# jean-pierreBoth/gsearch

Measured on AMD Instinct MI355X. Metric: query genomes/sec, higher is better.
Workload: dtype f32

## Files before the change

### gsearch_amd/csrc/gs_index.hip

```cpp
#include <algorithm>
#include <functional>
#include <chrono>
#include <math.h>
#include <memory>
#include <stdlib.h>
#include <string.h>
#include <vector>
#include <sys/stat.h>
#include "gs_internal.hpp"
#include "gs_spec.hpp"
#include "gs_insert_rows.hpp"
#include "gs_hnswio_parse.hpp"

namespace gs {

constexpr int ST = 1024;
constexpr int SMAXI = 16;
constexpr int RIF = 8;
#define KEY(c, id) (((uint64_t)(c) << 32) | (uint64_t)(id))
#define KCNT(k) ((uint32_t)((k) >> 32))
#define KID(k) ((uint32_t)(k))
#define INF_CNT 0xFFFFFFFFu

struct IndexDev {
// ... 1877 lines not shown
        list_ptrs(g, list, nbr, cnt, deg, cap);
        const uint32_t d = *deg, ni = inbox_cnt[list], n = d + ni;
        __syncthreads();
        for (uint32_t t = threadIdx.x; t < n; t += LM_T)
            keys[t] = t < d ? KEY(cnt[t], nbr[t]) : inbox[(uint64_t)list * inbox_cap + (t - d)];
        bool unsorted = false;
        for (uint32_t t = threadIdx.x + 1; t < d; t += LM_T) unsorted |= !(keys[t - 1] < keys[t]);
        const bool general = __syncthreads_or(unsorted) != 0;
        uint32_t rk[LM_MAX / LM_T]; uint64_t kv[LM_MAX / LM_T];
        uint32_t ndup = 0;
        if (general) {
            for (uint32_t t = threadIdx.x; t < n; t += LM_T) {
                const uint64_t k = keys[t]; uint32_t dup = 0;
                for (uint32_t j = 0; j < t; j++) dup |= (keys[j] == k);
                flag[t] = dup;
            }
            __syncthreads();
#pragma unroll
            for (int it = 0; it < LM_MAX / LM_T; it++) {
                const uint32_t t = threadIdx.x + it * LM_T;
                rk[it] = 0xFFFFFFFFu; kv[it] = 0;
                if (t < n && !flag[t]) {
                    const uint64_t k = keys[t]; uint32_t r = 0;
                    for (uint32_t j = 0; j < n; j++) r += (!flag[j] && keys[j] < k);
                    rk[it] = r; kv[it] = k;
                }
            }
            for (uint32_t j = 0; j < n; j++) ndup += flag[j];
        } else {
            for (uint32_t u = threadIdx.x; u < ni; u += LM_T) {
                const uint64_t k = keys[d + u];
                uint32_t lo = 0, hi = d;
                while (lo < hi) { const uint32_t mid = (lo + hi) >> 1; if (keys[mid] < k) lo = mid + 1; else hi = mid; }
                uint32_t dup = lo < d && keys[lo] == k;
                for (uint32_t v = 0; v < u; v++) dup |= (keys[d + v] == k);
                flag[d + u] = dup | (lo << 1);
            }
            __syncthreads();
#pragma unroll
            for (int it = 0; it < LM_MAX / LM_T; it++) {
                const uint32_t t = threadIdx.x + it * LM_T;
                rk[it] = 0xFFFFFFFFu; kv[it] = 0;
                if (t < d) {
                    const uint64_t k = keys[t]; uint32_t r = t;
                    for (uint32_t v = 0; v < ni; v++) r += (!(flag[d + v] & 1u) && keys[d + v] < k);
                    rk[it] = r; kv[it] = k;
                } else if (t < n && !(flag[t] & 1u)) {
                    const uint64_t k = keys[t]; uint32_t r = flag[t] >> 1;
                    for (uint32_t v = 0; v < ni; v++) r += (!(flag[d + v] & 1u) && keys[d + v] < k);
                    rk[it] = r; kv[it] = k;
                }
            }
            for (uint32_t v = 0; v < ni; v++) ndup += flag[d + v] & 1u;
        }
        __syncthreads();
#pragma unroll
        for (int it = 0; it < LM_MAX / LM_T; it++) if (rk[it] < cap) { nbr[rk[it]] = KID(kv[it]); cnt[rk[it]] = KCNT(kv[it]); }
        if (threadIdx.x == 0) { const uint32_t tot = n - ndup; *deg = tot < cap ? tot : cap; inbox_cnt[list] = 0; }
    }
}

}

struct gs_index {
    gs_ctx *ctx = nullptr;
    gs_index_params prm{};
    size_t esz = 4, rowbytes = 0; uint64_t stride = 0; uint32_t nchunks = 0;
    int ikind = GS_KIND_F32; size_t user_rowbytes = 0;
    uint64_t n = 0, cap = 0; int64_t entry = -1; int top = -1;
    uint64_t n_upper = 0, cap_upper = 0;
    gs::DevBuf data;
    gs::DevBuf levels;
    gs::DevBuf deg0;
    gs::DevBuf nbr0;
    gs::DevBuf cnt0;
    gs::DevBuf upidx;
    gs::DevBuf degU;
    gs::DevBuf nbrU;
    gs::DevBuf cntU;
    gs::DevBuf visited;
    gs::DevBuf counter;
    gs::DevBuf cbuf;
    gs::DevBuf blevels;
    gs::DevBuf cntmat;
    gs::DevBuf plan_keys;
    gs::DevBuf plan_n;
    gs::DevBuf inbox;
    gs::DevBuf inbox_cnt;
    gs::DevBuf touched;
    gs::DevBuf ntouched;
    gs::DevBuf evals_dev;
    gs::DevBuf wlog;
    gs::DevBuf w0_keys;
    gs::DevBuf w0_n;
    gs::DevBuf w0_evals;
    gs::DevBuf ep0;
    gs::DevBuf ext_keys;
    uint64_t inbox_lists = 0;
    uint64_t insert_evals = 0;
    gs::DevBuf mat;
    double search_frac = -1.0, insert_frac = -1.0;
    gs::DevBuf cols; uint64_t cols_cap = 0, cols_n = 0;
    gs::DevBuf join_scratch[gs::JOIN_SCRATCH];
    gs::DevBuf stats;
    uint64_t stat_wg_in_flight = 0, stat_adj_row_bytes = 0;
    gs::DevBuf rowptr;
    gs::DevBuf sp_off, sp_meta, sp_bm, sp_arena; uint32_t sp_L = 0; bool sp_tried = false;
    gs::VmArena sp_vm;
    bool sp_exhausted = false;
    uint64_t sp_reserved = 0;
    std::vector<std::unique_ptr<gs::DevBuf>> slabs;
    gs::DevBuf *call_slab = nullptr;
    gs::DevBuf *early_rows = nullptr;
    uint64_t pair_cache_bytes = 0, pair_cache_budget = 0;
    std::vector<uint64_t> origin;
    std::vector<int32_t> pid_rank;
    uint64_t level_count[17] = {0};
    gs::DevBuf origin_d, pid_rank_d; uint64_t origin_d_n = 0, pid_rank_d_n = 0;
    std::function<int(uint64_t, uint64_t)> *feed = nullptr; const uint8_t *feed_base = nullptr;
};

namespace gs {

static std::vector<DevBuf *> index_scratch(gs_index *ix)
{
    std::vector<DevBuf *> v = {&ix->visited, &ix->counter, &ix->cbuf, &ix->blevels, &ix->cntmat, &ix->plan_keys, &ix->plan_n, &ix->inbox, &ix->touched, &ix->ntouched,
                               &ix->wlog, &ix->w0_keys, &ix->w0_n, &ix->w0_evals, &ix->ep0, &ix->ext_keys, &ix->mat};
    for (DevBuf &b : ix->join_scratch) v.push_back(&b);
    return v;
}

static void ids_append(gs_index *ix, const uint64_t *ids, const uint8_t *lv, uint64_t n);

static void drop_pair_cache(gs_index *ix)
{
    (void)hipGetLastError();
    if (!ix->slabs.empty()) {
        (void)hipStreamSynchronize(ix->ctx->stream);
        if (ix->rowptr.p) (void)hipMemsetAsync(ix->rowptr.p, 0, ix->rowptr.bytes, ix->ctx->stream);
        (void)hipStreamSynchronize(ix->ctx->stream);
        ix->slabs.clear();
    }
    ix->call_slab = ix->early_rows = nullptr;
    ix->pair_cache_bytes = 0; ix->pair_cache_budget = 1;
}
static int alloc_or_evict(gs_index *ix, DevBuf &b, size_t bytes)
{
    int rc = b.alloc(bytes);
    if (rc == GS_OK || (ix->slabs.empty() && ix->pair_cache_budget == 1)) return rc;
    drop_pair_cache(ix);
    return b.alloc(bytes);
}

static int index_reserve(gs_index *ix, uint64_t need, uint64_t need_upper)
{
    gs_ctx *c = ix->ctx;
    const uint32_t M = ix->prm.max_nb_conn, ML = ix->prm.max_layer;
    if (need > ix->cap) {
        uint64_t ncap = std::max<uint64_t>(need, std::max<uint64_t>(ix->cap + ix->cap / 2, 1024));
        if (ix->prm.capacity >= need && ncap > ix->prm.capacity) ncap = ix->prm.capacity;
        if (ix->cols.p && (uint64_t)ix->stride * ncap > ((uint64_t)8 << 30)) { ix->cols.release(); ix->cols_cap = 0; ix->cols_n = 0; }
        struct Arr { DevBuf *b; size_t per; };
        std::vector<Arr> arr = {
            {&ix->data, (size_t)ix->stride}, {&ix->levels, 1}, {&ix->deg0, 4}, {&ix->nbr0, (size_t)8 * M}, {&ix->cnt0, (size_t)8 * M}, {&ix->upidx, 4}, {&ix->rowptr, 8}};
        if (ix->sp_L && ix->sp_meta.p) { arr.push_back({&ix->sp_off, 4}); arr.push_back({&ix->sp_meta, 8}); arr.push_back({&ix->sp_bm, 8}); }
        for (auto &a : arr) {
            DevBuf nb;
            int rc = alloc_or_evict(ix, nb, a.per * ncap); if (rc) return rc;
            GS_HIP_CHECK(hipMemsetAsync(nb.p, 0, a.per * ncap, c->stream));
            if (ix->n) GS_HIP_CHECK(hipMemcpyAsync(nb.p, a.b->p, a.per * ix->n, hipMemcpyDeviceToDevice, c->stream));
            GS_HIP_CHECK(hipStreamSynchronize(c->stream));
            std::swap(a.b->p, nb.p); std::swap(a.b->bytes, nb.bytes);
        }
        ix->cap = ncap;
    }
    if (need_upper > ix->cap_upper) {
        uint64_t ncap = std::max<uint64_t>(need_upper, std::max<uint64_t>(ix->cap_upper * 2, 64));
        struct { DevBuf *b; size_t per; } arr[] = {{&ix->degU, (size_t)4 * ML}, {&ix->nbrU, (size_t)4 * ML * M}, {&ix->cntU, (size_t)4 * ML * M}};
        for (auto &a : arr) {
            DevBuf nb;
            int rc = nb.alloc(a.per * ncap); if (rc) return rc;
            GS_HIP_CHECK(hipMemsetAsync(nb.p, 0, a.per * ncap, c->stream));
            if (ix->n_upper) GS_HIP_CHECK(hipMemcpyAsync(nb.p, a.b->p, a.per * ix->n_upper, hipMemcpyDeviceToDevice, c->stream));
            GS_HIP_CHECK(hipStreamSynchronize(c->stream));
            std::swap(a.b->p, nb.p); std::swap(a.b->bytes, nb.bytes);
        }
        ix->cap_upper = ncap;
    }
    return GS_OK;
}

static IndexDev index_dev(const gs_index *ix)
{
    IndexDev d;
    d.data = ix->data.as<uint8_t>(); d.stride = ix->stride; d.nchunks = ix->nchunks; d.m = ix->prm.m;
    d.M = ix->prm.max_nb_conn; d.max_layer = ix->prm.max_layer;
    d.levels = ix->levels.as<uint8_t>(); d.deg0 = ix->deg0.as<uint32_t>(); d.nbr0 = ix->nbr0.as<uint32_t>();
    d.upidx = ix->upidx.as<int32_t>(); d.degU = ix->degU.as<uint32_t>(); d.nbrU = ix->nbrU.as<uint32_t>();
    d.rowptr = ix->rowptr.as<uint64_t>();
    const bool sp = ix->sp_L && ix->sp_meta.p;
    d.sp_base = sp ? (const uint8_t *)ix->sp_vm.va : nullptr; d.sp_off = sp ? ix->sp_off.as<uint32_t>() : nullptr; d.sp_meta = sp ? ix->sp_meta.as<uint64_t>() : nullptr; d.sp_L = sp ? ix->sp_L : 0;
    d.sp_bm = sp ? ix->sp_bm.as<uint64_t>() : nullptr;
    d.n = ix->n; d.entry = ix->entry; d.top = ix->top;
    return d;
}

static int upload_rows(gs_ctx *c, void *dst, uint64_t stride, const void *src, size_t rowbytes, uint64_t nrows, hipMemcpyKind kind)
{
    if (nrows == 0) return GS_OK;
    GS_HIP_CHECK(hipMemsetAsync(dst, 0, stride * nrows, c->stream));
    GS_HIP_CHECK(hipMemcpy2DAsync(dst, stride, src, rowbytes, rowbytes, nrows, kind, c->stream));
    return GS_OK;
}

static int upload_user_rows(gs_index *ix, void *dst, const void *src, uint64_t nrows, hipMemcpyKind kind)
{
    gs_ctx *c = ix->ctx;
    if (ix->prm.kind != GS_KIND_U16) return upload_rows(c, dst, ix->stride, src, ix->rowbytes, nrows, kind);
    if (nrows == 0) return GS_OK;
    GS_HIP_CHECK(hipMemsetAsync(dst, 0, ix->stride * nrows, c->stream));
    const void *dev = src;
    PoolBuf stage(c, SL_IX_ROW_STAGE);
    if (kind == hipMemcpyHostToDevice) {
        int rc = stage.alloc(ix->user_rowbytes * nrows); if (rc) return rc;
        GS_HIP_CHECK(hipMemcpyAsync(stage.p, src, ix->user_rowbytes * nrows, hipMemcpyHostToDevice, c->stream));
        dev = stage.p;
    }
    return widen_u16_rows(c, dev, nrows, ix->prm.m, dst, ix->stride);
}
static int download_user_rows(gs_index *ix, uint64_t first, uint64_t n, void *out_host)
{
    gs_ctx *c = ix->ctx;
    if (n == 0) return GS_OK;
    if (ix->prm.kind != GS_KIND_U16) {
        GS_HIP_CHECK(hipMemcpy2DAsync(out_host, ix->rowbytes, ix->data.as<uint8_t>() + first * ix->stride, ix->stride, ix->rowbytes, n, hipMemcpyDeviceToHost, c->stream));
    } else {
        PoolBuf stage(c, SL_IX_ROW_STAGE);
        int rc = stage.alloc(ix->user_rowbytes * n); if (rc) return rc;
        if ((rc = narrow_u16_rows(c, ix->data.as<uint8_t>() + first * ix->stride, ix->stride, n, ix->prm.m, stage.p))) return rc;
        GS_HIP_CHECK(hipMemcpyAsync(out_host, stage.p, ix->user_rowbytes * n, hipMemcpyDeviceToHost, c->stream));
    }
    GS_HIP_CHECK(hipStreamSynchronize(c->stream));
    return GS_OK;
}

enum DistMode { MODE_AUTO = 0, MODE_GATHER = 1, MODE_DENSE = 2 };
static DistMode env_mode()
{
    const char *e = getenv("GS_DIST_MODE");
    if (!e) return MODE_AUTO;
    if (!strcmp(e, "gather")) return MODE_GATHER;
    if (!strcmp(e, "dense")) return MODE_DENSE;
    return MODE_AUTO;
}
static bool use_join(const gs_index *ix);
static bool dense_pays(const gs_index *ix, double frac, uint64_t nq)
{
    const double rc = ix->ctx->rel_compute, rh = ix->ctx->rel_hbm;
    const double n = (double)ix->n, q = (double)std::max<uint64_t>(nq, 1), evals = frac * n;
    const double gather = evals * (double)ix->rowbytes * std::max(q / (5.5e12 * rh), 1.0 / (8.0e10 * rh));
    double dense;
    if (use_join(ix)) dense = n * (double)ix->rowbytes / ((nq <= 512 ? 3.5e12 : 1.0e12) * rc) * std::ceil(q / (double)match_join_max_queries()) + 3e-3;
    else dense = std::ceil(q / 128.0) * 128.0 * n * (double)ix->prm.m / ((ix->ikind == GS_KIND_U64 ? 1.4e13 : 1.6e13) * rc);
    dense += evals * 75e-9 / rc * std::max(1.0, q / 768.0);
    return dense < gather;
}
static bool use_join(const gs_index *ix)
{
    const char *e = getenv("GS_DENSE_IMPL");
    if (e && !strcmp(e, "tile")) return false;
    return ix->prm.m <= 65535;
}
static int ensure_cols(gs_index *ix, uint64_t upto)
{
    gs_ctx *c = ix->ctx;
    int rc;
    if (ix->cols_cap != ix->cap || !ix->cols.p) {
        if ((rc = alloc_or_evict(ix, ix->cols, (size_t)ix->prm.m * ix->cap * ix->esz))) return rc;
        ix->cols_cap = ix->cap; ix->cols_n = 0;
    }
    if (ix->cols_n < upto) {
        if ((rc = rows_to_cols(c, ix->ikind, ix->prm.m, ix->data.as<uint8_t>() + ix->cols_n * ix->stride, ix->stride, upto - ix->cols_n, ix->cols.p, ix->cols_cap, ix->cols_n))) return rc;
        ix->cols_n = upto;
    }
    return GS_OK;
}
static int ensure_stats(gs_index *ix)
{
    if (ix->stats.p) return GS_OK;
    int rc = ix->stats.alloc(128);
    if (rc) return rc;
    GS_HIP_CHECK(hipMemsetAsync(ix->stats.p, 0, 128, ix->ctx->stream));
    return GS_OK;
}
static int dense_counts(gs_index *ix, const uint8_t *qrows, uint64_t nq, uint64_t n, uint16_t *out16, uint64_t ld)
{
    gs_ctx *c = ix->ctx;
    int rc;
    if (!use_join(ix))
        return hamming_qxc_strided(c, ix->ikind, ix->prm.m, qrows, nq, ix->stride, ix->data.p, n, ix->stride, nullptr, nullptr, out16, ld);
    if ((rc = ensure_cols(ix, n))) return rc;
    if ((rc = ensure_stats(ix))) return rc;
    const uint64_t parts = (nq + match_join_max_queries() - 1) / match_join_max_queries(), jq = (nq + parts - 1) / parts;
    for (uint64_t q0 = 0; q0 < nq; q0 += jq) {
        const uint64_t nb = std::min<uint64_t>(jq, nq - q0);
        int declined = 0;
        if (ix->feed && (rc = (*ix->feed)((uint64_t)(qrows - ix->feed_base) / ix->stride + q0, nb))) return rc;
        if ((rc = match_join_counts(c, ix->ikind, ix->prm.m, qrows + q0 * ix->stride, ix->stride, nb, ix->cols.p, ix->cols_cap, n, out16 + q0 * ld, ld, ix->join_scratch,
                                    &declined, ix->stats.as<unsigned long long>(), true, 0, ix->data.p, ix->stride))) return rc;
        if (declined &&
            (rc = hamming_qxc_strided(c, ix->ikind, ix->prm.m, qrows + q0 * ix->stride, nb, ix->stride, ix->data.p, n, ix->stride, nullptr, nullptr, out16 + q0 * ld, ld))) return rc;
    }
    return GS_OK;
}

static int dense_counts_range(gs_index *ix, const uint8_t *qrows, uint64_t nq, uint64_t node0, uint64_t nn, uint16_t *out16, uint64_t ld)
{
    gs_ctx *c = ix->ctx;
    int rc;
    if ((rc = ensure_cols(ix, node0 + nn))) return rc;
    if ((rc = ensure_stats(ix))) return rc;
    GS_REQUIRE(nq <= match_join_max_queries(), GS_ERR_INVALID, "dense_counts_range: too many rows");
    return match_join_counts(c, ix->ikind, ix->prm.m, qrows, ix->stride, nq, (const uint8_t *)ix->cols.p + node0 * ix->esz, ix->cols_cap, nn, out16, ld, ix->join_scratch,
                             nullptr, ix->stats.as<unsigned long long>(), false, node0);
}

static bool dense_vis_in_lds(const gs_index *ix, uint32_t knbn, uint32_t maxdeg)
{
    const size_t cap = 160 * 1024 - 1024;
    const size_t l = dense_lds_bytes(ix->prm.m, knbn, maxdeg, ix->n, true, maxdeg > (uint32_t)DT / 2 ? 512u : (uint32_t)DCN);
    const char *e = getenv("GS_DENSE_VIS");
    if (e && !strcmp(e, "global")) return false;
    if (e && !strcmp(e, "lds")) return l <= cap;
    return l <= cap;
}
static uint32_t dense_split_w(const gs_index *ix, uint32_t knbn, uint32_t maxdeg, uint32_t dcn, size_t min_bytes = 0, bool many_queries = false)
{
    const char *e = getenv("GS_DENSE_VIS");
    const bool forced = e && !strcmp(e, "split");
    if (e && !forced) { if (!strcmp(e, "global") || !strcmp(e, "lds")) return 0; }
    const bool one_per_cu = many_queries && round_up(dense_lds_bytes(ix->prm.m, knbn, maxdeg, ix->n, true, dcn), 1280) > (size_t)(160 * 1024 / 2);
    if (!forced && !one_per_cu && dense_vis_in_lds(ix, knbn, maxdeg)) return 0;
    const size_t base = std::max(dense_lds_bytes(ix->prm.m, knbn, maxdeg, 0, true, dcn), min_bytes);
    int per = getenv("GS_SPLIT_PER_CU") ? std::max(1, std::min(3, atoi(getenv("GS_SPLIT_PER_CU")))) : 2;
    uint64_t w = 0;
    for (; per >= 1 && w < 1024; per--) {
        const size_t budget = (size_t)(160 * 1024 / per) / 1280 * 1280 - 64;
        w = budget > base ? ((uint64_t)(budget - base) * 8) & ~(uint64_t)1023 : 0;
    }
    if (getenv("GS_SPLIT_W")) w = std::min<uint64_t>(w, (uint64_t)std::max(1024, atoi(getenv("GS_SPLIT_W"))) & ~(uint64_t)1023);
    if (w < 1024) return 0;
    return (uint32_t)std::min<uint64_t>(w, round_up(ix->n, 1024));
}
struct DenseGeom {
    bool ok;
    bool oneg, split, vlds;
    uint32_t dcn, vis_w;
    size_t lds;
    uint32_t per_cu, scratch_words, capC, grid;
    uint32_t p2_off;
};
static DenseGeom dense_geom(const gs_index *ix, uint64_t nq, uint32_t knbn, uint32_t ef, size_t min_lds_bytes, bool many_queries, bool with_log)
{
    const gs_ctx *c = ix->ctx;
    const size_t cap = 160 * 1024 - 1024;
    const uint32_t efs = std::max(ef, knbn), maxdeg = 2 * ix->prm.max_nb_conn;
    DenseGeom g{};
    g.oneg = maxdeg > (uint32_t)DT / 2;
    g.dcn = g.oneg ? 512u : (uint32_t)DCN;
    g.vis_w = dense_split_w(ix, knbn, maxdeg, g.dcn, min_lds_bytes, many_queries);
    g.split = g.vis_w != 0;
    const bool whole = dense_vis_in_lds(ix, knbn, maxdeg);
    g.vlds = with_log || g.split || whole;
    g.lds = std::max(dense_lds_bytes(ix->prm.m, knbn, maxdeg, g.split ? (uint64_t)g.vis_w : ix->n, g.vlds, g.dcn), min_lds_bytes);
    if (with_log && g.oneg) g.ok = false;
    else if (g.split) g.ok = true;
    else if (whole) g.ok = g.lds <= cap;
    else g.ok = !with_log && g.lds <= cap;
    const size_t granted = round_up(g.lds, 1280);
    g.per_cu = (uint32_t)std::max<size_t>(1, std::min<size_t>(3, (160 * 1024) / granted));
    if (g.oneg) g.per_cu = std::min<uint32_t>(g.per_cu, 2);
    if (!with_log && getenv("GS_DENSE_PER_CU")) g.per_cu = std::max(1, std::min((int)g.per_cu, atoi(getenv("GS_DENSE_PER_CU"))));
    g.scratch_words = (g.vlds ? dense_nblocks(ix->prm.m) * (HB / 2) : (uint32_t)((ix->n + 31) / 32)) + (g.split && ix->n > g.vis_w ? (uint32_t)((ix->n - g.vis_w + 31) / 32) : 0u);
    g.capC = 2 * efs + 2 * g.dcn + maxdeg + 64;
    g.grid = (uint32_t)std::min<uint64_t>(nq, (uint64_t)c->n_cu * g.per_cu);
    g.p2_off = (getenv("GS_DENSE_PHASE2") && !atoi(getenv("GS_DENSE_PHASE2"))) ? 1u : 0u;
    return g;
}
static int search_launch_dense(gs_index *ix, uint64_t nq, uint32_t knbn, uint32_t ef, const uint16_t *mat, uint64_t mat_ld, uint64_t *ids, float *dist,
                               uint32_t *count, uint64_t *evals)
{
    gs_ctx *c = ix->ctx;
    const DenseGeom g = dense_geom(ix, nq, knbn, ef, 0, nq >= (uint64_t)2 * c->n_cu, false);
    int rc;
    if ((rc = ensure_stats(ix))) return rc;
    ix->stat_wg_in_flight = g.grid; ix->stat_adj_row_bytes = (uint64_t)8 * ix->prm.max_nb_conn + 4;
    if ((rc = ix->visited.ensure((size_t)4 * g.scratch_words * c->n_cu * 3))) return rc;
    if ((rc = ix->cbuf.ensure((size_t)16 * g.capC * c->n_cu * 3))) return rc;
    GS_HIP_CHECK(hipMemsetAsync(ix->counter.p, 0, 8, c->stream));
    IndexDev d = index_dev(ix);
    unsigned long long *prof = nullptr;
    DevBuf profbuf;
    if (getenv("GS_TRAV_PROFILE")) { if ((rc = profbuf.alloc(128))) return rc; GS_HIP_CHECK(hipMemsetAsync(profbuf.p, 0, 128, c->stream)); prof = profbuf.as<unsigned long long>(); }
    {
    ProfScope ps(c, FAM_SEARCH);
#define GS_LAUNCH_DSEARCH(V, P, O, G) GS_LAUNCH_DSEARCH_S(V, P, O, G, false)
#define GS_LAUNCH_DSEARCH_S(V, P, O, G, SP)                                                                                  \
    do {                                                                                                                  \
        auto kern = k_hnsw_search_dense<V, P, O, G, false, SP>;                                                            \
        GS_HIP_CHECK(hipFuncSetAttribute((const void *)kern, hipFuncAttributeMaxDynamicSharedMemorySize, (int)g.lds));    \
        hipLaunchKernelGGL(kern, dim3(g.grid), dim3(DT), g.lds, c->stream, d, nq, knbn, ef, mat, mat_ld, ix->visited.as<uint32_t>(), g.scratch_words, \
                           ix->cbuf.as<uint64_t>(), g.capC, ix->counter.as<unsigned long long>(), ids, dist, count, evals, prof, ix->stats.as<unsigned long long>(),  \
                           (uint64_t *)nullptr, g.p2_off, 0u, (uint64_t *)nullptr, (uint32_t *)nullptr, (const uint32_t *)nullptr, g.vis_w);  \
    } while (0)
    if (g.split) { if (g.oneg) GS_LAUNCH_DSEARCH_S(true, false, 4, true, true); else GS_LAUNCH_DSEARCH_S(true, false, 4, false, true); }
    else if (g.oneg) { if (g.vlds) GS_LAUNCH_DSEARCH(true, false, 4, true); else GS_LAUNCH_DSEARCH(false, false, 4, true); }
    else if (prof) { if (g.vlds) GS_LAUNCH_DSEARCH(true, true, 4, false); else GS_LAUNCH_DSEARCH(false, true, 4, false); }
    else if (g.per_cu >= 3) { if (g.vlds) GS_LAUNCH_DSEARCH(true, false, 6, false); else GS_LAUNCH_DSEARCH(false, false, 6, false); }
    else { if (g.vlds) GS_LAUNCH_DSEARCH(true, false, 4, false); else GS_LAUNCH_DSEARCH(false, false, 4, false); }
#undef GS_LAUNCH_DSEARCH
#undef GS_LAUNCH_DSEARCH_S
    }
    GS_HIP_CHECK(hipGetLastError());
    if (prof) {
        unsigned long long h[16];
        GS_HIP_CHECK(hipMemcpyAsync(h, prof, 128, hipMemcpyDeviceToHost, c->stream));
        GS_HIP_CHECK(hipStreamSynchronize(c->stream));
        fprintf(stderr, "[GS_TRAV_PROFILE] workgroup 0: pops %llu merges %llu | cycles/pop: loads+atomics issue->ballot %.0f, sync1 %.0f, compaction+sync2 %.0f, accept rule+count %.0f | merge cycles/merge %.0f\n",
                h[5], h[6], (double)h[0] / h[5], (double)h[1] / h[5], (double)h[2] / h[5], (double)h[3] / h[5], h[6] ? (double)h[4] / h[6] : 0.0);
        if (h[6]) fprintf(stderr, "[GS_TRAV_PROFILE] of %llu accepting pops: %llu merged into T, %llu folded N into G\n", h[6], h[13], h[14]);
        if (h[6]) fprintf(stderr, "[GS_TRAV_PROFILE] per accepting pop: compaction+sort %.0f, prefetch+trim %.0f, T %.0f, fold+N merge %.0f cycles; accepted keys %.2f\n",
                          (double)h[8] / h[6], (double)h[9] / h[6], (double)h[10] / h[6], (double)h[11] / h[6], (double)h[12] / h[6]);
    }
    return GS_OK;
}

static bool dense_traversal_fits(const gs_index *ix, uint32_t knbn, uint32_t efs)
{
    const uint32_t maxdeg = 2 * ix->prm.max_nb_conn;
    return maxdeg <= (uint32_t)DT && efs <= 65535u && knbn <= (uint32_t)(TMAXI * DT) && ix->prm.m <= 65535u &&
           dense_lds_bytes(ix->prm.m, knbn, maxdeg, ix->n, false, maxdeg > (uint32_t)DT / 2 ? 512u : (uint32_t)DCN) <= 160 * 1024 - 1024 && !getenv("GS_DENSE_LEGACY");
}
static int search_launch(gs_index *ix, const uint8_t *q_padded_dev, uint64_t nq, uint32_t knbn, uint32_t ef, const uint16_t *mat, uint64_t mat_ld,
                         uint64_t *ids, float *dist, uint32_t *count, uint64_t *evals)
{
    gs_ctx *c = ix->ctx;
    const uint32_t efs = std::max(ef, knbn);
    const uint32_t maxdeg = 2 * ix->prm.max_nb_conn;
    if (mat && dense_traversal_fits(ix, knbn, efs)) return search_launch_dense(ix, nq, knbn, ef, mat, mat_ld, ids, dist, count, evals);
    const size_t lds = search_lds_bytes(efs, maxdeg);
    const uint32_t vis_words = (uint32_t)((ix->n + 31) / 32);
    uint32_t grid = (uint32_t)std::min<uint64_t>(nq, (uint64_t)c->n_cu);
    GS_HIP_CHECK(hipMemsetAsync(ix->counter.p, 0, 8, c->stream));
    IndexDev d = index_dev(ix);
    ProfScope ps(c, FAM_SEARCH);
#define GS_LAUNCH_SEARCH(K)                                                                                               \
    do {                                                                                                                  \
        auto kern = k_hnsw_search<K>;                                                                                     \
        GS_HIP_CHECK(hipFuncSetAttribute((const void *)kern, hipFuncAttributeMaxDynamicSharedMemorySize, (int)lds));      \
        hipLaunchKernelGGL(kern, dim3(grid), dim3(ST), lds, c->stream, d, q_padded_dev, nq, knbn, ef, mat, mat_ld,       \
                           ix->visited.as<uint32_t>(), vis_words, ix->counter.as<unsigned long long>(), ids, dist, count, evals); \
    } while (0)
    if (ix->ikind == GS_KIND_F32) GS_LAUNCH_SEARCH(GS_KIND_F32);
    else if (ix->ikind == GS_KIND_U32) GS_LAUNCH_SEARCH(GS_KIND_U32);
    else GS_LAUNCH_SEARCH(GS_KIND_U64);
#undef GS_LAUNCH_SEARCH
    GS_HIP_CHECK(hipGetLastError());
    return GS_OK;
}

static bool search_goes_dense(const gs_index *ix, uint64_t nq, uint32_t knbn, uint32_t ef)
{
    const uint32_t efs = std::max(ef, knbn);
    const DistMode mode = env_mode();
    if (ix->prm.m > 65535) return false;
    if (mode == MODE_DENSE) return true;
    const bool eligible = mode == MODE_AUTO && ix->n >= 4096;
    return eligible && dense_pays(ix, (double)std::min<uint64_t>(ix->n, efs) / (double)ix->n, nq);
}
static int search_dev(gs_index *ix, const void *q_padded_dev, uint64_t nq, uint32_t knbn, uint32_t ef, uint64_t *ids, float *dist,
                      uint32_t *count, uint64_t *evals)
{
    gs_ctx *c = ix->ctx;
    const uint32_t efs = std::max(ef, knbn);
    const uint32_t maxdeg = 2 * ix->prm.max_nb_conn;
    const size_t lds = search_lds_bytes(efs, maxdeg);
    GS_REQUIRE(maxdeg <= ST, GS_ERR_UNSUPPORTED, "max_nb_conn too large");
    const DistMode mode = env_mode();
    const bool fits_sorted = lds <= 160 * 1024 - 64 && 2 * (size_t)efs + maxdeg + 64 <= (size_t)SMAXI * ST;
    const bool dense_able = mode != MODE_GATHER && dense_traversal_fits(ix, knbn, efs);
    GS_REQUIRE(fits_sorted || dense_able, GS_ERR_UNSUPPORTED, "ef=%u needs %zu bytes of LDS in the sorted-array traversal (max ~%u with M=%u) and this index / mode does not admit the dense one (m <= 65535, ef <= 65535, GS_DIST_MODE != gather)",
               efs, lds, (unsigned)((160 * 1024 - 64 - 32 * maxdeg - 1024) / 24), ix->prm.max_nb_conn);
    const bool force_dense = !fits_sorted;
    const uint32_t vis_words = (uint32_t)((ix->n + 31) / 32);
    int rc;
    if ((rc = ix->visited.ensure((size_t)4 * vis_words * c->n_cu))) return rc;
    if ((rc = ix->counter.ensure(64))) return rc;
    const uint8_t *q = (const uint8_t *)q_padded_dev;
    uint64_t done = 0;
    DevBuf tmp_evals;
    const bool eligible = mode == MODE_AUTO && ix->prm.m <= 65535 && ix->n >= 4096;
    const bool lb_dense = eligible && dense_pays(ix, (double)std::min<uint64_t>(ix->n, efs) / (double)ix->n, nq);
    if (eligible && !lb_dense && ix->search_frac < 0 && nq >= 256 && !force_dense) {
        const uint64_t np = 128;
        uint64_t *ev = evals;
        if (!ev) { if ((rc = tmp_evals.alloc(8 * np))) return rc; ev = tmp_evals.as<uint64_t>(); }
        if ((rc = search_launch(ix, q, np, knbn, ef, nullptr, 0, ids, dist, count, ev))) return rc;
        std::vector<uint64_t> h(np);
        GS_HIP_CHECK(hipMemcpyAsync(h.data(), ev, 8 * np, hipMemcpyDeviceToHost, c->stream));
        GS_HIP_CHECK(hipStreamSynchronize(c->stream));
        double sum = 0; for (uint64_t v : h) sum += (double)v;
        ix->search_frac = sum / (double)np / (double)ix->n;
        done = np;
    }
    const uint64_t rest = nq - done;
    const double frac_known = ix->search_frac >= 0 ? ix->search_frac : ix->insert_frac;
    bool dense = ix->prm.m <= 65535 && (mode == MODE_DENSE || force_dense || lb_dense || (eligible && frac_known >= 0 && rest >= 1 && dense_pays(ix, frac_known, rest)));
    if (!dense) {
        if (rest) {
            uint64_t *ev = evals ? evals + done : nullptr;
            if (!ev && eligible && ix->search_frac < 0) { if ((rc = tmp_evals.alloc(8 * rest))) return rc; ev = tmp_evals.as<uint64_t>(); }
            if ((rc = search_launch(ix, q + done * ix->stride, rest, knbn, ef, nullptr, 0, ids + done * knbn, dist + done * knbn, count ? count + done : nullptr, ev))) return rc;
            if (eligible && ix->search_frac < 0 && ev) {
                const uint64_t ns = std::min<uint64_t>(rest, 128);
                std::vector<uint64_t> h(ns);
                GS_HIP_CHECK(hipMemcpyAsync(h.data(), ev, 8 * ns, hipMemcpyDeviceToHost, c->stream));
                GS_HIP_CHECK(hipStreamSynchronize(c->stream));
                double sum = 0; for (uint64_t v : h) sum += (double)v;
                ix->search_frac = sum / (double)ns / (double)ix->n;
            }
        }
        return GS_OK;
    }
    const uint64_t ld = round_up(ix->n, 8);
    const bool join = use_join(ix);
    uint64_t budget = (uint64_t)4 << 30;
    {
        size_t fr = 0, tot = 0;
        if (hipMemGetInfo(&fr, &tot) == hipSuccess) budget = std::max<uint64_t>(budget, std::min<uint64_t>((uint64_t)32 << 30, (uint64_t)(0.7 * (double)((uint64_t)fr + ix->mat.bytes))));
    }
    uint64_t QB = budget / (2 * ld);
    QB = std::max<uint64_t>(128, QB / 128 * 128);
    if (getenv("GS_SEARCH_QB")) QB = std::min<uint64_t>(QB, (uint64_t)std::max(1, atoi(getenv("GS_SEARCH_QB"))));
    QB = std::min<uint64_t>(QB, rest);
    const bool sv = getenv("GS_SEARCH_VERBOSE") != nullptr;
    const auto sv_t0 = std::chrono::steady_clock::now();
    if (sv) { size_t fr = 0, tot = 0; (void)hipMemGetInfo(&fr, &tot); fprintf(stderr, "[GS_SEARCH] nq %llu n %llu: QB %llu, count matrix %.2f GB wanted, %.2f GB held, device free %.2f GB\n", (unsigned long long)nq, (unsigned long long)ix->n, (unsigned long long)QB, 2.0 * QB * ld / 1e9, ix->mat.bytes / 1e9, fr / 1e9); }
    if (ix->mat.bytes < (size_t)2 * QB * ld && (rc = alloc_or_evict(ix, ix->mat, (size_t)2 * QB * ld))) return rc;
    if (sv) fprintf(stderr, "[GS_SEARCH] count matrix ready after %.1f ms\n", std::chrono::duration<double, std::milli>(std::chrono::steady_clock::now() - sv_t0).count());
    if (join && (rc = ensure_cols(ix, ix->n))) return rc;
    for (uint64_t q0 = done; q0 < nq; q0 += QB) {
        const uint64_t nb = std::min(QB, nq - q0);
        if ((rc = dense_counts(ix, q + q0 * ix->stride, nb, ix->n, ix->mat.as<uint16_t>(), ld))) return rc;
        if (sv) { (void)hipStreamSynchronize(c->stream); fprintf(stderr, "[GS_SEARCH] count matrix of %llu queries done at %.1f ms\n", (unsigned long long)nb, std::chrono::duration<double, std::milli>(std::chrono::steady_clock::now() - sv_t0).count()); }
        if ((rc = search_launch(ix, q + q0 * ix->stride, nb, knbn, ef, ix->mat.as<uint16_t>(), ld, ids + q0 * knbn, dist + q0 * knbn,
                                count ? count + q0 : nullptr, evals ? evals + q0 : nullptr))) return rc;
        if (sv) { (void)hipStreamSynchronize(c->stream); fprintf(stderr, "[GS_SEARCH] traversal done at %.1f ms\n", std::chrono::duration<double, std::milli>(std::chrono::steady_clock::now() - sv_t0).count()); }
    }
    return GS_OK;
}

}

extern "C" {

int gs_index_create(gs_ctx *c, const gs_index_params *p, gs_index **out)
{
    GS_REQUIRE(c && p && out, GS_ERR_INVALID, "null argument");
    GS_REQUIRE(p->kind == GS_KIND_F32 || p->kind == GS_KIND_U32 || p->kind == GS_KIND_U64 || p->kind == GS_KIND_U16, GS_ERR_UNSUPPORTED, "signature kind %d not supported by the index", p->kind);
    GS_REQUIRE(p->m >= 1, GS_ERR_INVALID, "m must be positive");
    GS_REQUIRE(p->max_nb_conn >= 2 && p->max_nb_conn <= 255, GS_ERR_INVALID, "max_nb_conn must be in 2..255 (gsearch.rs:268)");
    GS_REQUIRE(p->max_layer >= 1 && p->max_layer <= 16, GS_ERR_INVALID, "max_layer must be in 1..16");
    GS_REQUIRE(p->ef_construction >= 1, GS_ERR_INVALID, "ef_construction must be positive");
    gs_index *ix = new gs_index();
    ix->ctx = c; ix->prm = *p;
    if (ix->prm.insert_batch == 0) ix->prm.insert_batch = 64;
    ix->ikind = p->kind == GS_KIND_U16 ? GS_KIND_U32 : p->kind;
    ix->esz = gs::kind_bytes(ix->ikind);
    ix->rowbytes = ix->esz * p->m;
    ix->user_rowbytes = gs::kind_bytes(p->kind) * (size_t)p->m;
    ix->stride = gs::round_up(ix->rowbytes, 256);
    ix->nchunks = (uint32_t)((ix->rowbytes + 15) / 16);
    *out = ix;
    return GS_OK;
}
void gs_index_destroy(gs_index *ix)
{
    if (!ix) return;
    GS_CTX_LOCK(ix->ctx);
    (void)hipSetDevice(ix->ctx->device);
    (void)hipStreamSynchronize(ix->ctx->stream);
    delete ix;
}
uint64_t gs_index_nb_point(const gs_index *ix) { return ix ? ix->n : 0; }
int gs_index_search_stats(gs_index *ix, uint64_t out[8], int reset)
{
    GS_REQUIRE(ix && out, GS_ERR_INVALID, "null argument");
    gs_ctx *c = ix->ctx;
    GS_CTX_LOCK(c);
    for (int i = 0; i < 8; i++) out[i] = 0;
    if (ix->stats.p) {
        GS_HIP_CHECK(hipSetDevice(c->device));
        unsigned long long h[16];
        GS_HIP_CHECK(hipMemcpyAsync(h, ix->stats.p, 128, hipMemcpyDeviceToHost, c->stream));
        if (reset) GS_HIP_CHECK(hipMemsetAsync(ix->stats.p, 0, 128, c->stream));
        GS_HIP_CHECK(hipStreamSynchronize(c->stream));
// ... 1100 lines not shown
```

### gsearch_amd/csrc/gs_internal.hpp

```cpp
#pragma once
#include <hip/hip_runtime.h>
#include <stdint.h>
#include <stdio.h>
#include <algorithm>
#include <atomic>
#include <map>
#include <mutex>
#include <thread>
#include <string>
#include <vector>
#include "../../include/gsearch_amd.h"
#include "gs_scratch.hpp"
#include "gs_host.hpp"

namespace gs {

#define GS_HIP_CHECK(expr)                                                                         \
    do {                                                                                           \
        hipError_t _e = (expr);                                                                    \
        if (_e != hipSuccess) {                                                                    \
            gs::set_error("%s failed: %s (%s:%d)", #expr, hipGetErrorString(_e), __FILE__, __LINE__); \
            return GS_ERR_HIP;                                                                     \
        }                                                                                          \
    } while (0)

enum { FAM_SKETCH = 0, FAM_HAMMING = 1, FAM_SEARCH = 2, FAM_INSERT = 3, FAM_COUNT = 4 };

struct ProfSlot {
    std::vector<std::pair<hipEvent_t, hipEvent_t>> pending;
    double total_ms = 0;
    uint64_t launches = 0;
};

}

struct gs_ctx {
    int device = 0;
    hipStream_t stream = nullptr;
    bool own_stream = false;
    int n_cu = 0;
    uint64_t hbm_bytes = 0;
    double rel_compute = 1.0, rel_hbm = 1.0;
    char name[128] = {0};
    hipEvent_t t0 = nullptr, t1 = nullptr;
    bool profile = false;
    gs::ProfSlot prof[gs::FAM_COUNT];
    void *scratch_pool = nullptr;
    bool wait_sleeping = false;
    hipEvent_t sync_ev = nullptr;
    gs_ctx *child = nullptr;
    void *pinned_pool = nullptr;
    std::thread::id owner_thread{};
    std::map<std::thread::id, gs_ctx *> workers; std::mutex workers_mu;
    gs_ctx *parent = nullptr;
    uint64_t last_use = 0, use_tick = 0;
    int pins = 0; bool orphan = false;
    uint32_t last_sketch[4] = {0, 0, 0, 0};
    std::recursive_mutex mu;
};
#define GS_CTX_LOCK(c) std::lock_guard<std::recursive_mutex> gs_ctx_lock_((c)->mu); (void)hipSetDevice((c)->device)

namespace gs {

gs_ctx *worker_ctx(gs_ctx *c);
void worker_done(gs_ctx *parent, gs_ctx *worker);
void worker_unpin(gs_ctx *parent, gs_ctx *worker);
void on_worker_failed(gs_ctx *parent);
template <class F> inline int on_worker(gs_ctx *c, F &&body)
{
    gs_ctx *w = worker_ctx(c);
    int rc = body(w);
    if (w != c) {
        worker_done(c, w);
        if (rc == GS_ERR_HIP) { on_worker_failed(c); rc = body(c); }
    }
    return rc;
}

inline hipError_t stream_wait(gs_ctx *c)
{
    hipError_t e;
    if (!c->wait_sleeping) return hipStreamSynchronize(c->stream);
    if (!c->sync_ev && (e = hipEventCreateWithFlags(&c->sync_ev, hipEventBlockingSync | hipEventDisableTiming)) != hipSuccess) return e;
    if ((e = hipEventRecord(c->sync_ev, c->stream)) != hipSuccess) return e;
    return hipEventSynchronize(c->sync_ev);
}

struct ProfScope {
    gs_ctx *c; int fam; hipEvent_t a = nullptr, b = nullptr;
    ProfScope(gs_ctx *ctx, int family) : c(ctx), fam(family)
    {
        if (c->profile) {
            (void)hipEventCreate(&a); (void)hipEventCreate(&b);
            (void)hipEventRecord(a, c->stream);
        }
    }
    ~ProfScope()
    {
        if (c->profile) {
            (void)hipEventRecord(b, c->stream);
            c->prof[fam].pending.emplace_back(a, b);
        }
    }
};

int hamming_qxc_strided(gs_ctx *c, int kind, uint32_t m, const void *Q, uint64_t nq, uint64_t strideQ_bytes, const void *C, uint64_t nc,
                        uint64_t strideC_bytes, float *out, uint32_t *out_cnt, uint16_t *out_cnt16, uint64_t ld_out, uint32_t *parts_out = nullptr);

int widen_u16_rows(gs_ctx *c, const void *src_dev, uint64_t nrows, uint32_t m, void *dst_dev, uint64_t dst_stride_bytes);
int narrow_u16_rows(gs_ctx *c, const void *src_dev, uint64_t src_stride_bytes, uint64_t nrows, uint32_t m, void *dst_dev);

struct DevBuf;
uint64_t match_join_max_queries();
enum { JOIN_SCRATCH = 16 };
int match_join_counts(gs_ctx *c, int kind, uint32_t m, const void *qrows, uint64_t qstride, uint64_t nq, const void *cols, uint64_t colcap, uint64_t n,
                      uint16_t *out16, uint64_t ld, DevBuf *scratch, int *declined = nullptr, unsigned long long *stats = nullptr, bool init = true, uint64_t col0 = 0,
                      const void *rows = nullptr, uint64_t rstride = 0);
int hamming_blocks(gs_ctx *c, int kind, uint32_t m, const void *Q, uint64_t strideQ_bytes, const void *C, uint64_t strideC_bytes, const void *items_dev,
                   uint32_t n_items, const uint32_t *qlist_dev, const uint32_t *clist_dev, uint16_t *out_cnt16, uint64_t ld_out, uint32_t n_thin = 0,
                   uint32_t *parts_out = nullptr);
int rows_to_cols(gs_ctx *c, int kind, uint32_t m, const void *rows, uint64_t stride, uint64_t nrows, void *cols, uint64_t colcap, uint64_t first);

enum { KNN_MAX = 1024 };
int knn_select(gs_ctx *c, const uint16_t *mat, uint64_t ld, uint64_t nrows, uint64_t n, uint32_t knbn, uint32_t c_max, uint64_t diag0, uint32_t m,
               uint64_t *ids, float *dist, uint32_t *count);

struct ClusterSource {
    gs_index *ix = nullptr;
    uint64_t n = 0; uint32_t m = 0;
    uint64_t ld = 0;
    uint64_t max_rows = 0;
};
int cluster_rows(gs_index *ix, const uint32_t *nodes_dev, uint64_t nb, const uint16_t **slab);
int gather_rows(gs_ctx *c, const void *data, uint64_t stride, const uint32_t *nodes_dev, uint64_t nb, void *out);
int nearest_of_nodes(gs_ctx *c, const ClusterSource &src, const uint64_t *cand, uint64_t nc, uint32_t *arg_out, uint16_t *count_out);
int cluster_nodes(gs_ctx *c, const ClusterSource &src, const gs_cluster_params *prm, uint64_t *centre_node, uint16_t *centre_count, uint64_t *medoids,
                  uint64_t *sizes, uint64_t *core_nodes, uint64_t *core_weight, uint64_t core_cap, gs_cluster_info *info);

int embed_validate(gs_ctx *c, uint64_t n, uint32_t knbn, const uint64_t *ids, const float *dist, const uint32_t *cnt);
int embed_common(gs_ctx *c, bool on_dev, uint64_t n, uint32_t knbn, const uint64_t *dids, const float *ddist, const uint32_t *dcnt, const gs_embed_params *prm,
                 const float *init, float *pos_out, float *memb_out);
int knn_stats_dev(gs_ctx *c, uint64_t n, uint32_t knbn, const uint64_t *ids, const float *dist, const uint32_t *cnt, gs_knn_stats *st, uint32_t *occ_out,
                  uint64_t *hist_out);

int sketch_dev_impl(gs_ctx *c, const gs_sketch_params *p, const void *seq, uint64_t seq_bytes, const uint64_t *rec_start, const uint64_t *rec_len, uint64_t n_rec,
                    const uint64_t *genome_rec_off, uint64_t n_genomes, void *sig_out, bool sync_at_end);
int run_prob(gs_ctx *c, const gs_sketch_params *p, const uint8_t *seq, uint64_t seq_bytes, const uint64_t *rec_start, const uint64_t *rec_len, uint64_t n_rec,
             const uint64_t *genome_rec_off, uint64_t n_genomes, void *sig_out);
size_t radix_scratch_bytes(uint64_t n);
int radix_sort_u64(gs_ctx *c, uint64_t *keys, uint64_t *alt, uint64_t n, int endbit, void *scratch, uint64_t **sorted_out);
int run_length_encode_u64(gs_ctx *c, const uint64_t *sorted, uint64_t n, uint64_t *uniq, uint32_t *len, uint32_t *nruns_dev, uint32_t *pos, void *scratch);

inline size_t kind_bytes(int kind) { return kind == GS_KIND_U16 ? 2 : (kind == GS_KIND_U64 ? 8 : 4); }
inline uint64_t round_up(uint64_t x, uint64_t a) { return (x + a - 1) / a * a; }

inline std::atomic<int> debug_fill_byte{-1};
inline int debug_fill(void *p, size_t n)
{
    const int byte = debug_fill_byte.load(std::memory_order_relaxed);
    if (byte < 0 || !p || !n) return GS_OK;
    GS_HIP_CHECK(hipDeviceSynchronize());
    GS_HIP_CHECK(hipMemset(p, byte, n));
    GS_HIP_CHECK(hipDeviceSynchronize());
    return GS_OK;
}

inline bool mem_verbose() { static const bool v = getenv("GS_MEM_VERBOSE") != nullptr; return v; }
struct DevBuf {
    void *p = nullptr; size_t bytes = 0;
    DevBuf() = default;
    DevBuf(const DevBuf &) = delete;
    DevBuf &operator=(const DevBuf &) = delete;
    ~DevBuf() { release(); }
    void release() { if (p) { (void)hipFree(p); p = nullptr; bytes = 0; } }
    int alloc(size_t n)
    {
        release();
        if (n == 0) n = 16;
        const hipError_t e = hipMalloc(&p, n);
        if (e != hipSuccess || mem_verbose()) {
            size_t fr = 0, tot = 0;
            (void)hipMemGetInfo(&fr, &tot);
            if (e != hipSuccess) {
                p = nullptr;
                gs::set_error("hipMalloc of %zu bytes failed: %s (%zu of %zu bytes free on the device)", n, hipGetErrorString(e), fr, tot);
                return GS_ERR_HIP;
            }
            if (n >= ((size_t)256 << 20)) fprintf(stderr, "[GS_MEM] + %.2f GB (free after %.2f of %.2f GB)\n", n / 1e9, fr / 1e9, tot / 1e9);
        }
        bytes = n;
        return debug_fill(p, n);
    }
    int ensure(size_t n) { return (n <= bytes && p) ? GS_OK : alloc(n); }
    template <class T> T *as() const { return (T *)p; }
};

struct VmArena {
    size_t chunk = (size_t)1 << 30;
    void *va = nullptr; size_t va_bytes = 0, mapped = 0; int device = 0;
    std::vector<hipMemGenericAllocationHandle_t> handles;
    VmArena() = default;
    VmArena(const VmArena &) = delete;
    VmArena &operator=(const VmArena &) = delete;
    ~VmArena() { release(); }
    static bool supported(int dev)
    {
        int sup = 0;
        return hipDeviceGetAttribute(&sup, hipDeviceAttributeVirtualMemoryManagementSupported, dev) == hipSuccess && sup != 0;
    }
    bool reserve(int dev, size_t bytes, size_t chunk_bytes = (size_t)1 << 30)
    {
        release();
        if (!supported(dev)) return false;
        chunk = std::max<size_t>(chunk_bytes / 65536 * 65536, 65536);
        bytes = (bytes + chunk - 1) / chunk * chunk;
        if (hipMemAddressReserve(&va, bytes, 0, nullptr, 0) != hipSuccess) { (void)hipGetLastError(); va = nullptr; return false; }
        va_bytes = bytes; device = dev; mapped = 0;
        return true;
    }
    bool map_to(size_t bytes)
    {
        if (bytes > va_bytes) return false;
        hipMemAllocationProp prop = {};
        prop.type = hipMemAllocationTypePinned; prop.location.type = hipMemLocationTypeDevice; prop.location.id = device;
        hipMemAccessDesc acc = {};
        acc.location.type = hipMemLocationTypeDevice; acc.location.id = device; acc.flags = hipMemAccessFlagsProtReadWrite;
        while (mapped < bytes) {
            hipMemGenericAllocationHandle_t h;
            if (hipMemCreate(&h, chunk, &prop, 0) != hipSuccess) { (void)hipGetLastError(); return false; }
            if (hipMemMap((char *)va + mapped, chunk, 0, h, 0) != hipSuccess) { (void)hipGetLastError(); (void)hipMemRelease(h); return false; }
            if (hipMemSetAccess((char *)va + mapped, chunk, &acc, 1) != hipSuccess) { (void)hipGetLastError(); (void)hipMemUnmap((char *)va + mapped, chunk); (void)hipMemRelease(h); return false; }
            handles.push_back(h); mapped += chunk;
            if (mem_verbose()) fprintf(stderr, "[GS_MEM] arena: %.2f GB mapped of %.2f GB reserved\n", mapped / 1e9, va_bytes / 1e9);
        }
        return true;
    }
    void release()
    {
        for (size_t i = 0; i < handles.size(); i++) { (void)hipMemUnmap((char *)va + i * chunk, chunk); (void)hipMemRelease(handles[i]); }
        handles.clear();
        if (va) (void)hipMemAddressFree(va, va_bytes);
        va = nullptr; va_bytes = 0; mapped = 0;
    }
};

struct ScratchPool { DevBuf b[SCRATCH_SLOTS]; std::shared_ptr<SlotLeases> leases = std::make_shared<SlotLeases>(); };
inline void drop_scratch_pool(gs_ctx *c) { delete (ScratchPool *)c->scratch_pool; c->scratch_pool = nullptr; }
struct PinnedPool {
    void *p[PINNED_SLOTS] = {}; size_t cap[PINNED_SLOTS] = {};
    ~PinnedPool() { for (int i = 0; i < PINNED_SLOTS; i++) if (p[i]) (void)hipHostFree(p[i]); }
    void *ensure(int i, size_t n)
    {
        if (p[i] && cap[i] >= n) return p[i];
        if (p[i]) (void)hipHostFree(p[i]);
        p[i] = nullptr; cap[i] = 0;
        if (hipHostMalloc(&p[i], n, hipHostMallocDefault) != hipSuccess) { p[i] = nullptr; return nullptr; }
        cap[i] = n;
        return p[i];
    }
};
inline PinnedPool *pinned_pool(gs_ctx *c)
{
    if (!c->pinned_pool) c->pinned_pool = new PinnedPool();
    return (PinnedPool *)c->pinned_pool;
}
struct PoolBuf {
    gs_ctx *c; SlotLease lease; void *p = nullptr; size_t bytes = 0;
    PoolBuf(gs_ctx *ctx, ScratchSlot s) : c(ctx), lease(s) {}
    PoolBuf(const PoolBuf &) = delete;
    PoolBuf &operator=(const PoolBuf &) = delete;
    int alloc(size_t n)
    {
        if (!c->scratch_pool) c->scratch_pool = new ScratchPool();
        ScratchPool *pool = (ScratchPool *)c->scratch_pool;
        bool fresh = false;
        int rc = lease.take(pool->leases, &fresh);
        if (rc) return rc;
        DevBuf &d = pool->b[lease.slot];
        if (n == 0) n = 16;
        const bool grows = !(n <= d.bytes && d.p);
        if ((rc = d.ensure(n))) return rc;
        if (fresh && !grows && (rc = debug_fill(d.p, d.bytes))) return rc;
        p = d.p; bytes = n;
        return GS_OK;
    }
    void release() { lease.give(); p = nullptr; bytes = 0; }
    template <class T> T *as() const { return (T *)p; }
};

}
```

### gsearch_amd/csrc/gs_join.hip

```cpp
#include <string.h>
#include <algorithm>
#include <chrono>
#include <vector>
#include "gs_internal.hpp"
#include "gs_hamming_split.hpp"

namespace gs {

template <typename T> struct ElemKey;
template <> struct ElemKey<uint32_t> { static constexpr bool F = false; };

template <int KIND, typename T>
__device__ __forceinline__ T canon(T v)
{
    if (KIND == GS_KIND_F32) return (v == (T)0x80000000u) ? (T)0 : v;
    return v;
}
template <int KIND, typename T>
__device__ __forceinline__ bool never_equal(T v)
{
    if (KIND == GS_KIND_F32) return ((uint32_t)v & 0x7FFFFFFFu) > 0x7F800000u;
    return false;
}

template <typename T>
__global__ __launch_bounds__(256) void k_rows_to_cols(const uint8_t *__restrict__ rows, uint64_t stride, uint64_t nrows, uint32_t m, T *__restrict__ cols,
                                                       uint64_t colcap, uint64_t first, int f32)
{
    __shared__ T tile[32][33];
    const uint32_t tx = threadIdx.x & 31, ty = threadIdx.x >> 5;
    const uint64_t r0 = (uint64_t)blockIdx.x * 32, s0 = (uint64_t)blockIdx.y * 32;
    for (uint32_t j = ty; j < 32; j += 8) {
        const uint64_t r = r0 + j, s = s0 + tx;
        tile[j][tx] = (r < nrows && s < m) ? ((const T *)(rows + r * stride))[s] : (T)0;
    }
    __syncthreads();
    for (uint32_t j = ty; j < 32; j += 8) {
        const uint64_t s = s0 + j, r = r0 + tx;
        if (s < m && r < nrows) { const T v = tile[tx][j]; cols[s * colcap + first + r] = (f32 && v == (T)0x80000000u) ? (T)0 : v; }
    }
}

template <int KIND, typename T>
__global__ __launch_bounds__(256) void k_query_cols(const uint8_t *__restrict__ rows, uint64_t stride, uint32_t nq, uint32_t m, T *__restrict__ qkey)
{
    __shared__ T tile[32][33];
    const uint32_t tx = threadIdx.x & 31, ty = threadIdx.x >> 5;
    const uint64_t r0 = (uint64_t)blockIdx.x * 32, s0 = (uint64_t)blockIdx.y * 32;
    for (uint32_t j = ty; j < 32; j += 8) {
        const uint64_t r = r0 + j, s = s0 + tx;
        tile[j][tx] = (r < nq && s < m) ? ((const T *)(rows + r * stride))[s] : (T)0;
    }
    __syncthreads();
    for (uint32_t j = ty; j < 32; j += 8) {
        const uint64_t s = s0 + j, r = r0 + tx;
        if (s < m && r < nq) qkey[s * nq + r] = tile[tx][j];
    }
}

constexpr int JT = 1024;
constexpr int JU = 4;
constexpr int JP_MAX_LOG2 = 13;
constexpr int JQ_MAX = 3276;
constexpr int JB_LOG2 = 16;
constexpr uint32_t HTILE = HT;

__device__ __forceinline__ uint32_t join_hash(uint32_t k) { return k * 0x9E3779B1u; }
__device__ __forceinline__ uint32_t join_hash(uint64_t k) { return (uint32_t)((k * 0x9E3779B97F4A7C15ull) >> 32); }
#define GS_SEL4(a, i) (((i) & 2) ? (((i) & 1) ? a[3] : a[2]) : (((i) & 1) ? a[1] : a[0]))

#ifndef GS_JOIN_COUNT_KIND
#define GS_JOIN_COUNT_KIND 0
#endif
constexpr int JN = 8;
__device__ __forceinline__ void join_lds_barrier()
{
    __builtin_amdgcn_fence(__ATOMIC_RELEASE, "workgroup", "local");
    __builtin_amdgcn_s_barrier();
    __builtin_amdgcn_fence(__ATOMIC_ACQUIRE, "workgroup", "local");
}

__device__ __forceinline__ void join_wave_sync()
{
    __builtin_amdgcn_fence(__ATOMIC_RELEASE, "wavefront");
    __builtin_amdgcn_wave_barrier();
    __builtin_amdgcn_fence(__ATOMIC_ACQUIRE, "wavefront");
}

#define GS_JOIN_HIT(st, tagv, e)                                                                              \
    do {                                                                                                      \
        if (((st) & 0xFFFu) == (tagv)) (st) += 0x1000u;                                                       \
        else if ((st) < 0x2000u) { if (st) { join_flush(mm32, ld, (st), (e)); natom++; } (st) = (tagv) | 0x1000u; } \
        else { join_flush(mm32, ld, (tagv) | 0x1000u, (e)); natom++; }                                        \
    } while (0)
__device__ __forceinline__ void join_flush(uint32_t *mm32, uint64_t ld, uint32_t st, uint64_t e)
{
    const uint64_t idx = (uint64_t)((st & 0xFFFu) - 1) * ld + e;
    atomicSub(&mm32[idx >> 1], (st >> 12) << ((idx & 1) * 16));
}

constexpr uint32_t JTAG_MASK = 0xFFFu, JTAG_MULTI = 0x1000u, JTAG_MORE = 0x80000000u;
constexpr int JTAG_CL_SHIFT = 13;
constexpr uint32_t JCL_MAX = 2047;
constexpr int JWALK = 4;

template <int KIND, typename T, int SR, bool CL>
__global__ __launch_bounds__(JT, (sizeof(T) == 8 && SR == 1) ? 4 : 8) void k_match_join(const T *__restrict__ qkey, uint32_t nq, uint32_t log2p, const T *__restrict__ cols, uint64_t colcap, uint64_t n,
                                                    uint32_t slot_lo, uint32_t slot_hi, uint32_t slots_per_wg, uint32_t *__restrict__ mm32, uint64_t ld,
                                                    unsigned long long *__restrict__ stats, int chunk_major, uint64_t col0, const uint16_t *__restrict__ qcl,
                                                    const uint16_t *__restrict__ nodelab, const T *__restrict__ qs, uint32_t nh, const uint32_t *__restrict__ cl_lo,
                                                    const uint32_t *__restrict__ qlist, uint32_t dedup_flags)
{
    const uint32_t dedup_below = dedup_flags & 0x7FFFFFFFu;
    static_assert(JU == 4 && JN % JU == 0, "GS_SEL4 / pending mask are written for JU = 4");
    static_assert(!CL || SR == 1, "clusters: request batches only");
    constexpr bool E8 = sizeof(T) == 4 && SR == 1;
    constexpr bool DEDUP = CL && E8;
    constexpr bool D64 = sizeof(T) == 8 && SR == 1 && !CL;
    constexpr bool DENSE = E8 || D64;
    extern __shared__ __attribute__((aligned(16))) uint8_t s_raw[];
    const uint32_t P = 1u << log2p, mask = P - 1, sh = 32 - log2p;
    constexpr uint32_t BMW = (1u << JB_LOG2) / 32;
    uint32_t *tag = (uint32_t *)s_raw;
    uint32_t *bm = E8 ? (uint32_t *)(s_raw + 8 * (size_t)P) : (uint32_t *)(s_raw + 4 * (size_t)P * SR);
    T *key = (T *)(s_raw + (4 * (size_t)P + (size_t)BMW * 4) * SR);
    unsigned long long *ent = (unsigned long long *)s_raw;
    const uint32_t bchunk = chunk_major ? blockIdx.y : blockIdx.x, bslot = chunk_major ? blockIdx.x : blockIdx.y;
    const uint64_t e0 = (uint64_t)bchunk * (JT * JN) + threadIdx.x;
    const uint32_t s0 = slot_lo + bslot * slots_per_wg, s1 = s0 + slots_per_wg < slot_hi ? s0 + slots_per_wg : slot_hi;
    const uint2 *labT = CL ? (const uint2 *)nodelab + (uint64_t)bchunk * (JN / JU) * JT : nullptr;
    uint32_t sticky[JN];
    uint32_t natom = 0;
    uint32_t nexp = 0;
#pragma unroll
    for (int i = 0; i < JN; i++) sticky[i] = 0;
    const uint32_t lane = threadIdx.x & 63;
    uint32_t vmask = 0;
#pragma unroll
    for (int u = 0; u < JN; u++) vmask |= (uint32_t)(e0 + (uint64_t)u * JT < n) << u;
    const uint64_t ebase_u = col0 + (uint64_t)bchunk * (JT * JN);
    const uint32_t tid = threadIdx.x;
    uint32_t labmask = 0;
    if (CL && DENSE) {
#pragma unroll
        for (int it = 0; it < JN / JU; it++) {
            const uint2 l4 = labT[it * JT + threadIdx.x];
            labmask |= ((uint32_t)((l4.x & 0xFFFFu) != 0u) | (uint32_t)((l4.x >> 16) != 0u) << 1 | (uint32_t)((l4.y & 0xFFFFu) != 0u) << 2 | (uint32_t)((l4.y >> 16) != 0u) << 3) << (it * JU);
        }
    }
    const bool wave_lab = CL && DENSE && (dedup_flags >> 31) && __any(labmask != 0u);
    uint2 *wq = (uint2 *)(s_raw + (D64 ? 12 : 8) * (size_t)P + (size_t)BMW * 4) + (threadIdx.x >> 6) * (D64 ? 128 : 64);
    T vn[DENSE ? JN : JU];
#pragma unroll
    for (int u = 0; u < (DENSE ? JN : JU); u++) { const uint64_t e = e0 + (uint64_t)u * JT; vn[u] = (e < n && s0 < s1) ? cols[(uint64_t)s0 * colcap + e] : (T)0; }
    for (uint32_t sr = s0; sr < s1; sr += SR) {
        const uint32_t nr = s1 - sr < (uint32_t)SR ? s1 - sr : (uint32_t)SR;
        constexpr int JQ = DENSE ? (int)((((1u << JP_MAX_LOG2) * 2) / 5 + JT - 1) / JT) : 1;
        T kq[JQ];
        uint32_t tq[(JQ + 1) / 2] = {};
        if (DENSE) {
            typedef const T __attribute__((address_space(1))) *gptr;
            const uint64_t qb = (uint64_t)(qkey + (uint64_t)sr * nq);
            const gptr qk = (gptr)(((uint64_t)(uint32_t)__builtin_amdgcn_readfirstlane((uint32_t)(qb >> 32)) << 32) | (uint64_t)(uint32_t)__builtin_amdgcn_readfirstlane((uint32_t)qb));
            uint32_t o = threadIdx.x;
            asm volatile("" : "+v"(o));
#pragma unroll
            for (int j = 0; j < JQ; j++) { const gptr qj = qk + j * JT; kq[j] = o + (uint32_t)j * JT < nq ? qj[o] : (T)0; }
            if constexpr (CL) {
#pragma unroll
                for (int j = 0; j < JQ; j++) { const uint32_t i = o + (uint32_t)j * JT; tq[j >> 1] |= (i < nq ? (uint32_t)qcl[i] : 0u) << ((j & 1) * 16); }
            }
        }
        join_lds_barrier();
        if (E8) { for (uint32_t i = threadIdx.x; i < P; i += JT) ent[i] = 0ull; }
        else for (uint32_t i = threadIdx.x; i < P * SR; i += JT) tag[i] = 0;
        for (uint32_t i = threadIdx.x; i < BMW * SR; i += JT) bm[i] = 0;
        join_lds_barrier();
        auto insert_key = [&](const uint32_t r, const uint32_t q, T k, const uint32_t clq) {
            const uint32_t tw = CL ? (q + 1) | (clq << JTAG_CL_SHIFT) : q + 1;
            if (never_equal<KIND, T>(k)) return;
            k = canon<KIND, T>(k);
            const uint32_t hq = join_hash(k);
            atomicOr(&bm[r * BMW + (hq >> (32 - JB_LOG2 + 5))], (1u << ((hq >> (32 - JB_LOG2)) & 31)) | (1u << ((hq >> (27 - JB_LOG2)) & 31)));
            uint32_t h = hq >> sh;
            if (E8) {
                const unsigned long long nw = ((unsigned long long)tw << 32) | (uint32_t)k;
                for (;;) {
                    const unsigned long long old = atomicCAS(&ent[h], 0ull, nw);
                    if (old == 0ull) break;
                    if (DEDUP && (tw >> JTAG_CL_SHIFT) - 1u < dedup_below - 1u && (uint32_t)old == (uint32_t)k &&
                        (((uint32_t)(old >> 32) >> JTAG_CL_SHIFT) & JCL_MAX) == (tw >> JTAG_CL_SHIFT)) {
                        atomicOr((uint32_t *)&ent[h] + 1, JTAG_MULTI);
                        break;
                    }
                    if ((uint32_t)old == (uint32_t)k && !((uint32_t)(old >> 32) & JTAG_MORE)) atomicOr((uint32_t *)&ent[h] + 1, JTAG_MORE);
                    h = (h + 1) & mask;
                }
            } else {
                while (atomicCAS(&tag[r * P + h], 0u, tw) != 0u) h = (h + 1) & mask;
                key[r * P + h] = k;
            }
        };
        if (DENSE) {
#pragma unroll
            for (int j = 0; j < JQ; j++) { const uint32_t i = threadIdx.x + (uint32_t)j * JT; if (i < nq) insert_key(0u, i, kq[j], (tq[j >> 1] >> ((j & 1) * 16)) & 0xFFFFu); }
        } else {
            for (uint32_t i = threadIdx.x; i < nq * nr; i += JT) { const uint32_t r = i / nq, q = i - r * nq; insert_key(r, q, qkey[(uint64_t)(sr + r) * nq + q], CL ? (uint32_t)qcl[q] : 0u); }
        }
        uint2 lb0 = make_uint2(0u, 0u), lb1 = make_uint2(0u, 0u);
        if constexpr (CL && DENSE) {
            if (wave_lab) { uint32_t o0 = threadIdx.x, o1 = JT + threadIdx.x; asm volatile("" : "+v"(o0), "+v"(o1)); lb0 = labT[o0]; lb1 = labT[o1]; }
        }
        join_lds_barrier();
#pragma unroll 1
        for (uint32_t r = 0; r < nr; r++) {
            const uint32_t s = sr + r, tb = r * P, bb = r * BMW;
            const T *col = cols + (uint64_t)s * colcap;
            if constexpr (DENSE) {
                uint32_t pend = 0;
#pragma unroll
                for (int u0 = 0; u0 < JN; u0 += 4) {
                    uint32_t hsd[4], bwd[4];
#pragma unroll
                    for (int u = 0; u < 4; u++) { hsd[u] = join_hash(vn[u0 + u]); bwd[u] = bm[hsd[u] >> (32 - JB_LOG2 + 5)]; }
#pragma unroll
                    for (int u = 0; u < 4; u++) {
                        const uint32_t pass = (vmask >> (u0 + u)) & (bwd[u] >> ((hsd[u] >> (32 - JB_LOG2)) & 31)) & (bwd[u] >> ((hsd[u] >> (27 - JB_LOG2)) & 31)) & 1u;
                        pend |= pass << (u0 + u);
                    }
                }
                if constexpr (CL) {
                    if (wave_lab) {
#pragma unroll
                        for (int u = 0; u < JN; u++) {
                            const uint32_t l2 = u < 4 ? ((u & 2) ? lb0.y : lb0.x) : ((u & 2) ? lb1.y : lb1.x);
                            const uint32_t lab = (l2 >> ((u & 1) * 16)) & 0xFFFFu;
                            if (((pend >> u) & 1u) && lab != 0u) {
                                uint32_t hh = join_hash(vn[u]) >> sh;
#pragma unroll
                                for (int j = 0; j < JWALK; j++) {
                                    const unsigned long long en = ent[hh];
                                    const uint32_t t = (uint32_t)(en >> 32);
                                    if (t == 0u) { pend &= ~(1u << u); natom += GS_JOIN_COUNT_KIND == 8; break; }
                                    if ((uint32_t)en == (uint32_t)vn[u]) {
                                        if (((t >> JTAG_CL_SHIFT) & JCL_MAX) != lab) break;
                                        if (!(t & JTAG_MORE)) { pend &= ~(1u << u); natom += GS_JOIN_COUNT_KIND == 8; break; }
                                    }
                                    hh = (hh + 1) & mask;
                                }
                            }
                        }
                    }
                }
                while (__any(pend != 0u)) {
                    uint32_t qn = 0;
                    const uint32_t pend0 = pend;
#pragma unroll
                    for (int u = 0; u < JN; u++) {
                        const bool want = (pend >> u) & 1u;
                        const unsigned long long mw = __ballot(want);
                        const uint32_t cw = (uint32_t)__popcll(mw);
                        if (cw != 0u && qn + cw <= 64u) {
                            if (want) {
                                const uint32_t at = qn + __builtin_amdgcn_mbcnt_hi((uint32_t)(mw >> 32), __builtin_amdgcn_mbcnt_lo((uint32_t)mw, 0u));
                                const uint32_t who = lane | ((uint32_t)u << 6) | (sticky[u] << 9) | (CL ? ((labmask >> u) & 1u) << 29 : 0u);
                                if constexpr (D64) { wq[2 * at] = make_uint2((uint32_t)vn[u], (uint32_t)((uint64_t)vn[u] >> 32)); wq[2 * at + 1].x = who; }
                                else wq[at] = make_uint2((uint32_t)vn[u], who);
                            }
                            qn += cw; pend &= ~(1u << u);
                        }
                    }
                    join_wave_sync();
                    if constexpr (CL) {
                        if (GS_JOIN_COUNT_KIND == 7 && lane < qn) natom++;
                        bool have = lane < qn;
                        uint2 qe = make_uint2(0u, 0u);
                        if (have) qe = wq[lane];
                        uint32_t st = (qe.y >> 9) & 0xFFFFFu, flp = 0;
                        const uint32_t eloc = (qe.y & 63u) + ((qe.y >> 6) & 7u) * JT;
                        uint32_t hh = join_hash((T)qe.x) >> sh;
                        for (;;) {
                            uint32_t mitem = 0;
                            if (have) {
                                const unsigned long long en = ent[hh];
                                const uint32_t t = (uint32_t)(en >> 32);
                                if (t == 0u) have = false;
                                else {
                                    if ((uint32_t)en == qe.x) {
                                        if (!(t & JTAG_MORE)) have = false;
                                        bool count_it = true;
                                        if ((t >> 12) & 0x7FFFFu) {
                                            const uint32_t cl = (t >> JTAG_CL_SHIFT) & JCL_MAX;
                                            uint32_t nl = 0;
                                            if ((qe.y >> 29) & 1u) {
                                                const uint32_t uo = (qe.y >> 6) & 7u, to = threadIdx.x - lane + (qe.y & 63u);
                                                nl = nodelab[(((uint64_t)bchunk * (JN / JU) + (uo >> 2)) * JT + to) * JU + (uo & 3u)];
                                            }
                                            if (nl == cl) { count_it = false; natom += GS_JOIN_COUNT_KIND == 9; }
                                            else if (t & JTAG_MULTI) { mitem = cl; count_it = false; }
                                        }
                                        if (count_it) {
                                            const uint32_t tg = t & JTAG_MASK, one = tg | 0x1000u;
                                            const bool same = (st & 0xFFFu) == tg, weak = st < 0x2000u, full = st >= 0xFF000u;
                                            const uint32_t fl = same ? (full ? st : 0u) : (weak ? st : one);
                                            st = same ? (full ? one : st + 0x1000u) : (weak ? one : st);
                                            if (fl) {
                                                if (flp) { join_flush(mm32, ld, flp, ebase_u + (tid - lane + eloc)); natom += GS_JOIN_COUNT_KIND == 0; }
                                                flp = fl;
                                            }
                                        }
                                    }
                                    hh = (hh + 1) & mask;
                                }
                            }
                            unsigned long long pm = __ballot(mitem != 0u);
                            while (pm) {
                                const int src = __ffsll((long long)pm) - 1;
                                pm &= pm - 1;
                                nexp++;
                                const uint32_t cl = __builtin_amdgcn_readlane(mitem, src), vsrc = __builtin_amdgcn_readlane(qe.x, src);
                                const uint64_t e = ebase_u + (tid - lane + __builtin_amdgcn_readlane(eloc, src));
                                const uint32_t lo = cl_lo[cl], hi = cl_lo[cl + 1];
                                for (uint32_t pos = lo + lane; pos < hi; pos += 64) {
                                    const T k2 = qs[(uint64_t)s * nh + pos];
                                    if (!never_equal<KIND, T>(k2) && (uint32_t)canon<KIND, T>(k2) == vsrc) {
                                        const uint64_t idx = (uint64_t)qlist[pos] * ld + e;
                                        atomicSub(&mm32[idx >> 1], 1u << ((idx & 1) * 16));
                                        natom += GS_JOIN_COUNT_KIND == 0;
                                    }
                                }
                            }
                            if (!__any(have)) break;
                        }
                        if (lane < qn) {
                            if (flp) { join_flush(mm32, ld, flp, ebase_u + (tid - lane + eloc)); natom += GS_JOIN_COUNT_KIND == 0; }
                            wq[lane].x = st;
                        }
                    } else if constexpr (D64) {
                        if (lane < qn) {
                            const uint2 q0 = wq[2 * lane];
                            const uint32_t who = wq[2 * lane + 1].x;
                            const T val = (T)((uint64_t)q0.x | ((uint64_t)q0.y << 32));
                            uint32_t st = who >> 9, flp = 0;
                            const uint32_t eo = (who & 63u) + ((who >> 6) & 7u) * JT - lane;
                            uint32_t hh = join_hash(val) >> sh;
                            for (;;) {
                                const uint32_t t = tag[hh];
                                if (t == 0u) break;
                                if (key[hh] == val) {
                                    const uint32_t tg = t & JTAG_MASK, one = tg | 0x1000u;
                                    const bool same = (st & 0xFFFu) == tg, weak = st < 0x2000u, full = st >= 0xFF000u;
                                    const uint32_t fl = same ? (full ? st : 0u) : (weak ? st : one);
                                    st = same ? (full ? one : st + 0x1000u) : (weak ? one : st);
                                    if (fl) {
                                        if (flp) { join_flush(mm32, ld, flp, ebase_u + (tid + eo)); natom++; }
                                        flp = fl;
                                    }
                                }
                                hh = (hh + 1) & mask;
                            }
                            if (flp) { join_flush(mm32, ld, flp, ebase_u + (tid + eo)); natom++; }
                            wq[2 * lane + 1].x = st;
                        }
                    } else
                    if (lane < qn) {
                        const uint2 qe = wq[lane];
                        uint32_t st = qe.y >> 9, flp = 0;
                        const uint32_t eo = (qe.y & 63u) + ((qe.y >> 6) & 7u) * JT - lane;
                        uint32_t hh = join_hash((T)qe.x) >> sh;
                        for (;;) {
                            const unsigned long long en = ent[hh];
                            const uint32_t t = (uint32_t)(en >> 32);
                            if (t == 0u) break;
                            if ((uint32_t)en == qe.x) {
                                const uint32_t tg = t & JTAG_MASK, one = tg | 0x1000u;
                                const bool same = (st & 0xFFFu) == tg, weak = st < 0x2000u, full = st >= 0xFF000u;
                                const uint32_t fl = same ? (full ? st : 0u) : (weak ? st : one);
                                if (GS_JOIN_COUNT_KIND == 1 && !same && !weak) natom++;
                                if (GS_JOIN_COUNT_KIND == 2 && !same && weak && st) natom++;
                                if (GS_JOIN_COUNT_KIND == 5) natom++;
                                if (GS_JOIN_COUNT_KIND == 6 && same) natom++;
                                st = same ? (full ? one : st + 0x1000u) : (weak ? one : st);
                                if (fl) {
                                    if (flp) { join_flush(mm32, ld, flp, ebase_u + (tid + eo)); natom += GS_JOIN_COUNT_KIND == 0; }
                                    flp = fl;
                                }
                                if (!(t & JTAG_MORE)) break;
                            }
                            hh = (hh + 1) & mask;
                        }
                        if (flp) { join_flush(mm32, ld, flp, ebase_u + (tid + eo)); natom += GS_JOIN_COUNT_KIND == 0; }
                        wq[lane].x = st;
                    }
                    join_wave_sync();
                    const uint32_t queued = pend0 & ~pend;
                    uint32_t qb = 0;
#pragma unroll
                    for (int u = 0; u < JN; u++) {
                        const bool mine = (queued >> u) & 1u;
                        const unsigned long long mw = __ballot(mine);
                        if (mw != 0ull) {
                            if (mine) { const uint32_t at = qb + __builtin_amdgcn_mbcnt_hi((uint32_t)(mw >> 32), __builtin_amdgcn_mbcnt_lo((uint32_t)mw, 0u)); sticky[u] = D64 ? wq[2 * at + 1].x : wq[at].x; }
                            qb += (uint32_t)__popcll(mw);
                        }
                    }
                    join_wave_sync();
                }
                if (s + 1 < s1) {
                    const uint64_t cb = (uint64_t)(col + colcap + (uint64_t)bchunk * (JT * JN));
                    typedef const T __attribute__((address_space(1))) *gptr;
                    const gptr cn = (gptr)(((uint64_t)(uint32_t)__builtin_amdgcn_readfirstlane((uint32_t)(cb >> 32)) << 32) | (uint64_t)(uint32_t)__builtin_amdgcn_readfirstlane((uint32_t)cb));
#pragma unroll
                    for (int u = 0; u < JN; u++) { const gptr cu = cn + u * JT; vn[u] = ((vmask >> u) & 1u) ? __builtin_nontemporal_load(cu + threadIdx.x) : (T)0; }
                }
            } else {
#pragma unroll
            for (int it = 0; it < JN / JU; it++) {
                uint2 lab4 = make_uint2(0u, 0u);
                if (CL) { uint32_t o = it * JT + threadIdx.x; asm volatile("" : "+v"(o)); lab4 = labT[o]; }
                T v[JU]; uint32_t hs[JU]; uint32_t pend = 0; uint32_t bw[JU];
#pragma unroll
                for (int u = 0; u < JU; u++) {
                    v[u] = canon<KIND, T>(vn[u]);
                    hs[u] = join_hash(v[u]);
                    bw[u] = bm[bb + (hs[u] >> (32 - JB_LOG2 + 5))];
                }
#pragma unroll
                for (int u = 0; u < JU; u++) {
                    const uint64_t e = e0 + (uint64_t)(it * JU + u) * JT;
                    const uint32_t bit = hs[u] >> (32 - JB_LOG2);
                    const uint32_t pass = (uint32_t)(e < n) & (uint32_t)!never_equal<KIND, T>(vn[u]) & (bw[u] >> (bit & 31)) & (bw[u] >> ((hs[u] >> (27 - JB_LOG2)) & 31)) & 1u;
                    pend |= pass << u;
                }
#pragma unroll
                for (int u = 0; u < JU; u++) {
                    const bool wrap = it + 1 == JN / JU;
                    const uint64_t e = e0 + (uint64_t)((wrap ? 0 : (it + 1) * JU) + u) * JT;
                    const T *src = wrap ? col + colcap : col;
                    vn[u] = (e < n && (!wrap || s + 1 < s1)) ? src[e] : (T)0;
                }
                uint32_t hh = 0, uu = 0; T vv = 0; bool have = false;
                {
                for (;;) {
                    if (!have && pend) { uu = (uint32_t)__ffs((int)pend) - 1; pend &= pend - 1; vv = GS_SEL4(v, uu); hh = GS_SEL4(hs, uu) >> sh; have = true; }
                    if (!have) break;
                    uint32_t t; T k;
                    if (E8) { const unsigned long long en = ent[hh]; t = (uint32_t)(en >> 32); k = (T)(uint32_t)en; }
                    else { t = tag[tb + hh]; k = key[tb + hh]; }
                    if (t == 0u) { have = false; continue; }
                    if (k == vv) {
                        if (E8 && !(t & JTAG_MORE)) have = false;
                        const uint32_t ni = it * JU + uu;
                        const uint64_t el = e0 + (uint64_t)ni * JT;
                        bool count_it = true;
                        if (CL && ((t >> 12) & 0x7FFFFu))
                            count_it = (((uu & 2u ? lab4.y : lab4.x) >> ((uu & 1u) * 16)) & 0xFFFFu) != ((t >> JTAG_CL_SHIFT) & JCL_MAX);
                        if (count_it) {
                            const uint64_t e = col0 + el;
                            uint32_t st = GS_SEL4((sticky + it * JU), uu);
                            GS_JOIN_HIT(st, t & JTAG_MASK, e);
#pragma unroll
                            for (int u = 0; u < JU; u++) if (uu == (uint32_t)u) sticky[it * JU + u] = st;
                        }
                    }
                    hh = (hh + 1) & mask;
                }
                }
            }
            }
        }
    }
#pragma unroll
    for (int i = 0; i < JN; i++) if (sticky[i]) { join_flush(mm32, ld, sticky[i], ebase_u + (tid + (uint32_t)i * JT)); natom += GS_JOIN_COUNT_KIND == 0 || (GS_JOIN_COUNT_KIND == 3 && sticky[i] >= 0x2000u) || (GS_JOIN_COUNT_KIND == 4 && sticky[i] < 0x2000u); }
    if (stats) {
#pragma unroll
        for (int o = 32; o > 0; o >>= 1) natom += __shfl_down(natom, o);
        if ((threadIdx.x & 63) == 0 && natom) atomicAdd(stats, (unsigned long long)natom);
        if (CL && (threadIdx.x & 63) == 0 && nexp) atomicAdd(stats + 7, (unsigned long long)nexp);
    }
}
template <int KIND, typename T>
__global__ __launch_bounds__(JT) void k_match_sample(const T *__restrict__ qkey, uint32_t nq, uint32_t log2p, const T *__restrict__ cols, uint64_t colcap, uint64_t n,
                                                      uint32_t m, uint32_t nsamp, unsigned long long *__restrict__ out)
{
    extern __shared__ __attribute__((aligned(16))) uint8_t s_raw[];
    const uint32_t P = 1u << log2p, mask = P - 1, sh = 32 - log2p;
    uint32_t *tag = (uint32_t *)s_raw;
    T *key = (T *)(s_raw + 4 * (size_t)P);
    const uint64_t e0 = (uint64_t)blockIdx.x * (JT * JN) + threadIdx.x;
    const uint32_t sbase = (uint32_t)(((uint64_t)blockIdx.y * (m - 1)) / nsamp);
    uint32_t first[JN];
#pragma unroll
    for (int i = 0; i < JN; i++) first[i] = 0;
    uint32_t hits = 0, reps = 0;
    for (uint32_t pass = 0; pass < 2; pass++) {
        const uint32_t s = sbase + pass;
        __syncthreads();
        for (uint32_t i = threadIdx.x; i < P; i += JT) tag[i] = 0;
        __syncthreads();
        for (uint32_t q = threadIdx.x; q < nq; q += JT) {
            T k = qkey[(uint64_t)s * nq + q];
            if (never_equal<KIND, T>(k)) continue;
            k = canon<KIND, T>(k);
            uint32_t h = join_hash(k) >> sh;
            while (atomicCAS(&tag[h], 0u, q + 1) != 0u) h = (h + 1) & mask;
            key[h] = k;
        }
        __syncthreads();
#pragma unroll
        for (int i = 0; i < JN; i++) {
            const uint64_t e = e0 + (uint64_t)i * JT;
            if (e >= n) continue;
            T v = cols[(uint64_t)s * colcap + e];
            if (never_equal<KIND, T>(v)) continue;
            v = canon<KIND, T>(v);
            uint32_t h = join_hash(v) >> sh, t;
            while ((t = tag[h]) != 0u) {
                if (key[h] == v) {
                    if (pass == 0) { if (!first[i]) first[i] = t; }
                    else { hits++; reps += (t == first[i]); }
                }
                h = (h + 1) & mask;
            }
        }
    }
#pragma unroll
    for (int o = 32; o > 0; o >>= 1) { hits += __shfl_down(hits, o); reps += __shfl_down(reps, o); }
    if ((threadIdx.x & 63) == 0 && hits) { atomicAdd(&out[0], (unsigned long long)hits); atomicAdd(&out[1], (unsigned long long)reps); }
}

constexpr uint32_t JS0 = 48, JHEAVY = 3;
constexpr uint64_t JPAIR_CAP = (uint64_t)4 << 20, JPAIR_MAX = (uint64_t)256 << 20;
constexpr uint32_t JTILE_CAP = 24576;
constexpr uint32_t JDEDUP_MINQ = 2;

constexpr uint32_t HS_STAGE = 3072;
__global__ __launch_bounds__(256) void k_heavy_scan(const uint16_t *__restrict__ mat, uint64_t ld, uint32_t nq, uint64_t n, uint32_t m, uint2 *__restrict__ pairs,
                                                    unsigned long long *__restrict__ ctr , uint64_t cap)
{
    __shared__ uint2 stage[HS_STAGE];
    __shared__ uint32_t sn;
    __shared__ unsigned long long sbase;
    if (threadIdx.x == 0) sn = 0;
    __syncthreads();
    const uint64_t tiles_per_row = (n + 2047) / 2048, ntiles = tiles_per_row * nq;
    uint32_t tot = 0;
    auto flush = [&]() {
        __syncthreads();
        const uint32_t cnt = sn;
        if (cnt) {
            if (threadIdx.x == 0) sbase = atomicAdd(&ctr[0], (unsigned long long)cnt);
            __syncthreads();
            const unsigned long long base = sbase;
            for (uint32_t i = threadIdx.x; i < cnt; i += 256) if (base + i < cap) pairs[base + i] = stage[i];
            __syncthreads();
            if (threadIdx.x == 0) sn = 0;
        }
        __syncthreads();
    };
    for (uint64_t t = blockIdx.x; t < ntiles; t += gridDim.x) {
        const uint32_t q = (uint32_t)(t / tiles_per_row);
        const uint64_t e8 = (t - (uint64_t)q * tiles_per_row) * 2048 + (uint64_t)threadIdx.x * 8;
        if (e8 < n) {
            const uint4 w = *(const uint4 *)(mat + (uint64_t)q * ld + e8);
            const uint32_t ww[4] = {w.x, w.y, w.z, w.w};
#pragma unroll
            for (int i = 0; i < 8; i++) {
                const uint32_t c = (ww[i >> 1] >> ((i & 1) * 16)) & 0xFFFFu;
                const uint32_t def = (e8 + i < n) ? m - c : 0u;
                tot += def;
                if (def >= JHEAVY) stage[atomicAdd(&sn, 1u)] = make_uint2((uint32_t)(e8 + i), q | (def << 16));
            }
        }
        __syncthreads();
        if (sn >= HS_STAGE - 2048) flush();
    }
    flush();
#pragma unroll
    for (int o = 32; o > 0; o >>= 1) tot += __shfl_down(tot, o);
    if ((threadIdx.x & 63) == 0 && tot) atomicAdd(&ctr[1], (unsigned long long)tot);
}
__global__ void k_label_init(uint32_t *__restrict__ labq, uint32_t nq, uint32_t *__restrict__ labe, uint64_t n)
{
    const uint64_t i = (uint64_t)blockIdx.x * blockDim.x + threadIdx.x;
    if (i < nq) labq[i] = (uint32_t)i;
    if (i < n) labe[i] = 0xFFFFFFFFu;
}
__global__ void k_label_prop(const uint2 *__restrict__ pairs, const unsigned long long *__restrict__ ctr, uint64_t cap, uint32_t *__restrict__ labq, uint32_t *__restrict__ labe)
{
    const uint64_t np = ctr[0] < cap ? ctr[0] : cap;
    for (uint64_t i = (uint64_t)blockIdx.x * blockDim.x + threadIdx.x; i < np; i += (uint64_t)gridDim.x * blockDim.x) {
        const uint2 p = pairs[i];
        const uint32_t q = p.y & 0xFFFFu, a = labq[q], b = labe[p.x], l = a < b ? a : b;
        if (l < a) atomicMin(&labq[q], l);
        if (l < b) atomicMin(&labe[p.x], l);
    }
}
__global__ void k_label_count(const uint32_t *__restrict__ labe, uint64_t n, uint32_t nq, uint32_t *__restrict__ cnt)
{
    for (uint64_t e = (uint64_t)blockIdx.x * blockDim.x + threadIdx.x; e < n; e += (uint64_t)gridDim.x * blockDim.x) { const uint32_t l = labe[e]; if (l < nq) atomicAdd(&cnt[l], 1u); }
}
template <typename T>
__global__ __launch_bounds__(256) void k_query_cols_list(const uint8_t *__restrict__ rows, uint64_t stride, const uint32_t *__restrict__ qlist, uint32_t nh, uint32_t m, T *__restrict__ qs)
{
    __shared__ T tile[32][33];
    const uint32_t tx = threadIdx.x & 31, ty = threadIdx.x >> 5;
    const uint64_t r0 = (uint64_t)blockIdx.x * 32, s0 = (uint64_t)blockIdx.y * 32;
    for (uint32_t j = ty; j < 32; j += 8) {
        const uint64_t r = r0 + j, s = s0 + tx;
        tile[j][tx] = (r < nh && s < m) ? ((const T *)(rows + (uint64_t)qlist[r] * stride))[s] : (T)0;
    }
    __syncthreads();
    for (uint32_t j = ty; j < 32; j += 8) {
        const uint64_t s = s0 + j, r = r0 + tx;
        if (s < m && r < nh) qs[s * nh + r] = tile[tx][j];
    }
}
struct JoinGeom { uint32_t chunks, log2p; size_t lds1, ldsq; };

template <int KIND, typename T, bool CL>
static int join_launch(gs_ctx *c, const JoinGeom &g, const T *qkey, uint32_t nq, const void *cols, uint64_t colcap, uint64_t n, uint32_t slot_lo, uint32_t slot_hi,
                       uint16_t *out16, uint64_t ld, unsigned long long *stats, uint64_t col0, bool few_blocks, const uint16_t *qcl, const uint16_t *nodelab, const T *qs,
                       uint32_t nh, const uint32_t *cl_lo, const uint32_t *qlist, uint32_t dedup_below = 0)
{
    const uint32_t ms = slot_hi - slot_lo, chunks = g.chunks;
    uint32_t blocks = std::max<uint32_t>(1, std::min<uint32_t>((16 * c->n_cu) / chunks, std::max<uint32_t>(ms / 32, (2 * c->n_cu) / chunks)));
    if (few_blocks) blocks = std::max<uint32_t>(1, std::min<uint32_t>(ms / 4, (2 * c->n_cu + chunks - 1) / chunks));
    if (getenv("GS_JOIN_BLOCKS") && !few_blocks) blocks = (uint32_t)atoi(getenv("GS_JOIN_BLOCKS"));
    blocks = std::min<uint32_t>(std::max<uint32_t>(blocks, 1), ms);
    const uint32_t slots_per_wg = (ms + blocks - 1) / blocks;
    const int chunk_major = getenv("GS_JOIN_CHUNK_MAJOR") ? atoi(getenv("GS_JOIN_CHUNK_MAJOR")) : ((nq >= 1024 && chunks >= 16) ? 1 : 0);
    const uint32_t nblk = (ms + slots_per_wg - 1) / slots_per_wg;
    dim3 jg(chunk_major ? nblk : chunks, chunk_major ? chunks : nblk);
    int sr = 1;
    if (!CL) {
        if (4 * g.lds1 <= 80 * 1024 && slots_per_wg >= 8) sr = 4; else if (2 * g.lds1 <= 80 * 1024 && slots_per_wg >= 4) sr = 2;
        if (getenv("GS_JOIN_SLOTS_PER_ROUND")) { const int e = atoi(getenv("GS_JOIN_SLOTS_PER_ROUND")); if (e == 1 || (e == 2 && 2 * g.lds1 <= 80 * 1024) || (e == 4 && 4 * g.lds1 <= 80 * 1024)) sr = e; }
    }
    const size_t lds = g.lds1 * sr + (sr == 1 ? g.ldsq : 0);
    ProfScope ps(c, FAM_HAMMING);
#define GS_JOIN_GO(KERN)                                                                                                                              \
    do {                                                                                                                                              \
        auto kern = KERN;                                                                                                                             \
        if (lds > 48 * 1024) GS_HIP_CHECK(hipFuncSetAttribute((const void *)kern, hipFuncAttributeMaxDynamicSharedMemorySize, (int)lds));             \
        hipLaunchKernelGGL(kern, jg, dim3(JT), lds, c->stream, qkey, nq, g.log2p, (const T *)cols, colcap, n, slot_lo, slot_hi, slots_per_wg, (uint32_t *)out16, ld, \
                           stats, chunk_major, col0, qcl, nodelab, qs, nh, cl_lo, qlist, dedup_below);                                                             \
    } while (0)
    if (CL) GS_JOIN_GO((k_match_join<KIND, T, 1, CL>));
    else if (sr == 4) GS_JOIN_GO((k_match_join<KIND, T, 4, false>));
    else if (sr == 2) GS_JOIN_GO((k_match_join<KIND, T, 2, false>));
    else GS_JOIN_GO((k_match_join<KIND, T, 1, false>));
#undef GS_JOIN_GO
    GS_HIP_CHECK(hipGetLastError());
    return GS_OK;
}

template <int KIND, typename T>
static int join_sample_declines(gs_ctx *c, const JoinGeom &g, uint32_t m, const T *qkey, uint32_t nq, const void *cols, uint64_t colcap, uint64_t n, DevBuf *scratch, int *decline_out)
{
    int rc;
    const uint32_t nsamp = 24;
    DevBuf &cnt = scratch[1];
    if ((rc = cnt.ensure(16))) return rc;
    GS_HIP_CHECK(hipMemsetAsync(cnt.p, 0, 16, c->stream));
    const size_t lds_s = (sizeof(T) + 4) * ((size_t)1 << g.log2p);
    auto ks = k_match_sample<KIND, T>;
    if (lds_s > 48 * 1024) GS_HIP_CHECK(hipFuncSetAttribute((const void *)ks, hipFuncAttributeMaxDynamicSharedMemorySize, (int)lds_s));
    hipLaunchKernelGGL(ks, dim3(g.chunks, nsamp), dim3(JT), lds_s, c->stream, qkey, nq, g.log2p, (const T *)cols, colcap, n, m, nsamp, cnt.as<unsigned long long>());
    GS_HIP_CHECK(hipGetLastError());
    unsigned long long hr[2] = {0, 0};
    GS_HIP_CHECK(hipMemcpyAsync(hr, cnt.p, 16, hipMemcpyDeviceToHost, c->stream));
    GS_HIP_CHECK(hipStreamSynchronize(c->stream));
    const double scale = (double)m / (double)nsamp;
    const double atomics = (double)(hr[0] - hr[1]) * scale + (double)hr[1] * scale / 64.0;
    const double t_join = (double)n * m * sizeof(T) / 3.5e12 + atomics / 1.6e10 + (double)hr[0] * scale / 2.0e11;
    const double t_tile = (double)((nq + 127) / 128 * 128) * (double)n * (double)m / (KIND == GS_KIND_U64 ? 1.4e13 : 1.6e13);
    const char *force = getenv("GS_JOIN_DECLINE");
    const bool decline = force ? atoi(force) != 0 : t_join > t_tile;
    if (getenv("GS_JOIN_VERBOSE"))
        fprintf(stderr, "[GS_JOIN] nq=%u n=%llu sampled matches %llu repeats %llu -> est. join %.2f ms, tile %.2f ms: %s\n", nq, (unsigned long long)n, hr[0], hr[1],
                t_join * 1e3, t_tile * 1e3, decline ? "tile" : "join");
    *decline_out = decline ? 1 : 0;
    return GS_OK;
}

template <int KIND, typename T>
static int join_impl(gs_ctx *c, uint32_t m, const uint8_t *qrows, uint64_t qstride, uint32_t nq, const void *cols, uint64_t colcap, uint64_t n, uint16_t *out16,
                     uint64_t ld, DevBuf *scratch , int *declined, unsigned long long *stats, bool init, uint64_t col0,
                     const void *rows, uint64_t rstride)
{
    int rc;
    if (declined) *declined = 0;
    const size_t items = (size_t)m * nq;
    DevBuf &k0 = scratch[0];
    if ((rc = k0.ensure(sizeof(T) * items))) return rc;
    if (init) GS_HIP_CHECK(hipMemsetD16Async((hipDeviceptr_t)out16, (unsigned short)m, (size_t)nq * ld, c->stream));
    dim3 tg((nq + 31) / 32, (m + 31) / 32);
    hipLaunchKernelGGL((k_query_cols<KIND, T>), tg, dim3(256), 0, c->stream, qrows, qstride, nq, m, k0.as<T>());
    GS_HIP_CHECK(hipGetLastError());
    JoinGeom g;
    g.log2p = 6;
    while (g.log2p < (uint32_t)JP_MAX_LOG2 && (double)(1u << g.log2p) * 0.4 < (double)nq) g.log2p++;
    g.chunks = (uint32_t)((n + (uint64_t)JT * JN - 1) / ((uint64_t)JT * JN));
    g.lds1 = (sizeof(T) + 4) * ((size_t)1 << g.log2p) + ((size_t)1 << JB_LOG2) / 8;
    g.ldsq = (size_t)(JT / 64) * 64 * (sizeof(T) == 4 ? 8 : 16);
    const bool may_decline = declined && m >= 64 && n >= 4096;
    const char *ce = getenv("GS_JOIN_CLUSTER");
    bool cluster = declined && init && col0 == 0 && rows && nq >= 256 && n >= 8192 && m >= 16 * JS0 && (ld % 8) == 0 && !(ce && !atoi(ce)) && !getenv("GS_JOIN_DECLINE");
    if (ce && atoi(ce) == 2) cluster = declined && init && col0 == 0 && rows && m >= 2 * JS0 && (ld % 8) == 0;
    if (!cluster) {
        if (may_decline) {
            int dec = 0;
            if ((rc = join_sample_declines<KIND, T>(c, g, m, k0.as<T>(), nq, cols, colcap, n, scratch, &dec))) return rc;
            if (dec) { *declined = 1; return GS_OK; }
        }
        return join_launch<KIND, T, false>(c, g, k0.as<T>(), nq, cols, colcap, n, 0, m, out16, ld, stats, col0, false, nullptr, nullptr, nullptr, 0, nullptr, nullptr);
    }
    const bool verbose = getenv("GS_JOIN_VERBOSE") != nullptr;
    const bool times = getenv("GS_JOIN_TIMES") != nullptr;
    auto t_prev = std::chrono::steady_clock::now();
    auto lap = [&](const char *what) {
        if (!times) return;
        (void)hipStreamSynchronize(c->stream);
        const auto now = std::chrono::steady_clock::now();
        fprintf(stderr, "[GS_JOIN_TIMES] %-28s %8.3f ms\n", what, std::chrono::duration<double, std::milli>(now - t_prev).count());
        t_prev = now;
    };
    lap("query columns + memset");
    DevBuf &pairs = scratch[2], &ctr = scratch[3], &labq = scratch[4], &labe = scratch[5];
    uint64_t pair_cap = JPAIR_CAP;
    DevBuf &lcnt = scratch[14];
    if ((rc = pairs.ensure(pair_cap * 8)) || (rc = ctr.ensure(64)) || (rc = labq.ensure(4 * (size_t)nq)) || (rc = labe.ensure(4 * (size_t)n)) || (rc = lcnt.ensure(4 * (size_t)nq))) return rc;
    pair_cap = std::max<uint64_t>(pair_cap, pairs.bytes / 8);
    if ((rc = join_launch<KIND, T, false>(c, g, k0.as<T>(), nq, cols, colcap, n, 0, JS0, out16, ld, stats, 0, true, nullptr, nullptr, nullptr, 0, nullptr, nullptr))) return rc;
    lap("phase 0 (first slots)");
    uint8_t *pin = (uint8_t *)pinned_pool(c)->ensure(PIN_JOIN, 64 + 4 * (2 * (size_t)nq + n) + 2 * ((size_t)nq + 8 + (size_t)g.chunks * JT * JN) + 64);
    GS_REQUIRE(pin, GS_ERR_HIP, "match-join: pinned staging buffer");
    unsigned long long *hc = (unsigned long long *)pin;
    uint32_t *hlq = (uint32_t *)(pin + 64), *hcn = hlq + nq, *hle = hcn + nq;
    for (int attempt = 0;; attempt++) {
        GS_HIP_CHECK(hipMemsetAsync(ctr.p, 0, 64, c->stream));
        hipLaunchKernelGGL(k_heavy_scan, dim3(c->n_cu * 8), dim3(256), 0, c->stream, out16, ld, nq, n, m, pairs.as<uint2>(), ctr.as<unsigned long long>(), pair_cap);
        lap("heavy scan");
        hipLaunchKernelGGL(k_label_init, dim3((uint32_t)((std::max<uint64_t>(n, nq) + 255) / 256)), dim3(256), 0, c->stream, labq.as<uint32_t>(), nq, labe.as<uint32_t>(), n);
        for (int it = 0; it < 6; it++)
            hipLaunchKernelGGL(k_label_prop, dim3(c->n_cu * 4), dim3(256), 0, c->stream, pairs.as<uint2>(), ctr.as<unsigned long long>(), pair_cap, labq.as<uint32_t>(), labe.as<uint32_t>());
        GS_HIP_CHECK(hipMemsetAsync(lcnt.p, 0, 4 * (size_t)nq, c->stream));
        hipLaunchKernelGGL(k_label_count, dim3(c->n_cu * 2), dim3(256), 0, c->stream, labe.as<uint32_t>(), n, nq, lcnt.as<uint32_t>());
        GS_HIP_CHECK(hipGetLastError());
        GS_HIP_CHECK(hipMemcpyAsync(hc, ctr.p, 16, hipMemcpyDeviceToHost, c->stream));
        GS_HIP_CHECK(hipMemcpyAsync(hlq, labq.p, 4 * (size_t)nq, hipMemcpyDeviceToHost, c->stream));
        GS_HIP_CHECK(hipMemcpyAsync(hcn, lcnt.p, 4 * (size_t)nq, hipMemcpyDeviceToHost, c->stream));
        GS_HIP_CHECK(hipStreamSynchronize(c->stream));
        lap("labels + query labels down");
        if (hc[0] <= pair_cap || attempt || hc[0] > JPAIR_MAX) break;
        if (pairs.alloc((size_t)hc[0] * 8 + 4096) != GS_OK) { (void)hipGetLastError(); (void)pairs.alloc(JPAIR_CAP * 8); pair_cap = JPAIR_CAP; break; }
        pair_cap = hc[0] + 512;
    }
    const uint64_t npairs = hc[0];
    std::vector<uint32_t> cq(nq, 0), ce_(nq, 0), cid(nq, 0);
    uint32_t K = 0, ntiles = 0, nhq = 0, dedup_below = 1;
    uint64_t nhe = 0;
    const uint32_t minq = getenv("GS_JOIN_CLUSTER_MINQ") ? (uint32_t)std::max(2, atoi(getenv("GS_JOIN_CLUSTER_MINQ"))) : (ce && atoi(ce) == 2 ? 2u : 12u);
    const uint64_t minpairs = getenv("GS_JOIN_CLUSTER_MINPAIRS") ? (uint64_t)atoll(getenv("GS_JOIN_CLUSTER_MINPAIRS")) : 128;
    auto is_cluster = [&](uint32_t l) { return cq[l] >= minq || (cq[l] >= 2 && (uint64_t)(cq[l] - 1) * hcn[l] >= minpairs); };
    const uint64_t min_scaled0 = (uint64_t)((double)nq * 32.0 * (double)n / 3.0e5);
    const uint64_t min_saved0 = getenv("GS_JOIN_CLUSTER_MIN") ? (uint64_t)atoll(getenv("GS_JOIN_CLUSTER_MIN")) : (ce && atoi(ce) == 2 ? 0 : std::max<uint64_t>((uint64_t)nq * 8, min_scaled0));
    bool any = false;
    if (npairs <= pair_cap) {
        for (uint32_t q = 0; q < nq; q++) if (hlq[q] < nq) ++cq[hlq[q]];
        uint64_t est = 0;
        for (uint32_t l = 0; l < nq; l++) if (cq[l] && hcn[l] && is_cluster(l)) { any = true; est += (uint64_t)(cq[l] - 1) * hcn[l]; }
        if (est < min_saved0) any = false;
    }
    if (any) {
        GS_HIP_CHECK(hipMemcpyAsync(hle, labe.p, 4 * (size_t)n, hipMemcpyDeviceToHost, c->stream));
        GS_HIP_CHECK(hipStreamSynchronize(c->stream));
        for (uint64_t e = 0; e < n; e++) if (hle[e] < nq) ce_[hle[e]]++;
        std::vector<uint32_t> order;
        for (uint32_t l = 0; l < nq; l++) if (ce_[l] >= 1 && is_cluster(l)) order.push_back(l);
        auto tiles_of = [&](uint32_t l) { return ((cq[l] + HTILE - 1) / HTILE) * ((ce_[l] + HTILE - 1) / HTILE); };
        std::sort(order.begin(), order.end(), [&](uint32_t a, uint32_t b) { const uint32_t ta = tiles_of(a), tb = tiles_of(b); return ta != tb ? ta < tb : a < b; });
        std::vector<uint32_t> chosen;
        for (uint32_t l : order) {
            if (chosen.size() >= JCL_MAX || ntiles + tiles_of(l) > JTILE_CAP) break;
            chosen.push_back(l); ntiles += tiles_of(l); nhq += cq[l]; nhe += ce_[l];
        }
        const uint32_t dq = getenv("GS_JOIN_DEDUP_MINQ") ? (uint32_t)std::max(2, atoi(getenv("GS_JOIN_DEDUP_MINQ"))) : JDEDUP_MINQ;
        std::stable_sort(chosen.begin(), chosen.end(), [&](uint32_t a, uint32_t b) { return (cq[a] >= dq) > (cq[b] >= dq); });
        for (uint32_t l : chosen) { cid[l] = ++K; if (cq[l] >= dq) dedup_below = K + 1; }
    }
    uint64_t saved_pairs = 0;
    for (uint32_t l = 0; l < nq; l++) if (cid[l]) saved_pairs += (uint64_t)(cq[l] - 1) * ce_[l];
    const uint64_t min_scaled = (uint64_t)((double)nq * 32.0 * (double)n / 3.0e5);
    const uint64_t min_saved = getenv("GS_JOIN_CLUSTER_MIN") ? (uint64_t)atoll(getenv("GS_JOIN_CLUSTER_MIN")) : (ce && atoi(ce) == 2 ? 0 : std::max<uint64_t>((uint64_t)nq * 8, min_scaled));
    if (verbose)
        fprintf(stderr, "[GS_JOIN] nq=%u n=%llu heavy pairs %llu (matches in the first %u slots %llu): %u clusters, %u queries x %llu nodes in %u tiles, %llu pairs off the atomics%s\n", nq,
                (unsigned long long)n, (unsigned long long)npairs, JS0, hc[1], K, nhq, (unsigned long long)nhe, ntiles, (unsigned long long)saved_pairs,
                K && saved_pairs < min_saved ? " - not worth the cluster-aware pass" : "");
    if (K && saved_pairs < min_saved) K = 0;
    lap("host: components");
    if (K == 0) {
        const double t_tile = (double)((nq + 127) / 128 * 128) * (double)n * (double)m / (KIND == GS_KIND_U64 ? 1.4e13 : 1.6e13);
        if (may_decline && (npairs > pair_cap || (double)hc[1] * ((double)m / JS0) / 1.6e10 > 0.5 * t_tile)) {
            int dec = 0;
            if ((rc = join_sample_declines<KIND, T>(c, g, m, k0.as<T>(), nq, cols, colcap, n, scratch, &dec))) return rc;
            if (dec) { *declined = 1; return GS_OK; }
        }
        return join_launch<KIND, T, false>(c, g, k0.as<T>(), nq, cols, colcap, n, JS0, m, out16, ld, stats, 0, false, nullptr, nullptr, nullptr, 0, nullptr, nullptr);
    }
    std::vector<uint32_t> cl_lo(K + 2, 0), ce_lo(K + 2, 0);
    for (uint32_t l = 0; l < nq; l++) if (cid[l]) { cl_lo[cid[l] + 1] = cq[l]; ce_lo[cid[l] + 1] = ce_[l]; }
    for (uint32_t k = 1; k <= K + 1; k++) { cl_lo[k] += cl_lo[k - 1]; ce_lo[k] += ce_lo[k - 1]; }
    std::vector<uint32_t> qlist(nhq), elist(nhe), fq(cl_lo.begin(), cl_lo.end()), fe(ce_lo.begin(), ce_lo.end());
    const uint64_t npad = (uint64_t)g.chunks * JT * JN;
    uint16_t *hqcl = (uint16_t *)(hle + n), *hnl = hqcl + ((nq + 3) & ~3u);
    for (uint32_t q = 0; q < nq; q++) { const uint32_t l = hlq[q]; hqcl[q] = 0; if (l < nq && cid[l]) { hqcl[q] = (uint16_t)cid[l]; qlist[fq[cid[l]]++] = q; } }
    memset(hnl, 0, 2 * npad);
    for (uint64_t e = 0; e < n; e++) {
        const uint32_t l = hle[e];
        if (l < nq && cid[l]) {
            const uint64_t ch = e / (JT * JN), w = e % (JT * JN), i = w / JT, ln = w % JT;
            hnl[((ch * (JN / JU) + i / JU) * JT + ln) * JU + i % JU] = (uint16_t)cid[l];
            elist[fe[cid[l]]++] = (uint32_t)e;
        }
    }
    std::vector<uint4> tiles;
    tiles.reserve(ntiles);
    uint32_t n_thin = 0;
    for (int pass = 0; pass < 2; pass++)
        for (uint32_t k = 1; k <= K; k++)
            for (uint32_t a = cl_lo[k]; a < cl_lo[k + 1]; a += HTILE) {
                const uint32_t qr = std::min<uint32_t>(HTILE, cl_lo[k + 1] - a);
                if ((qr <= (uint32_t)HTQ) != (pass == 0)) continue;
                for (uint32_t b = ce_lo[k]; b < ce_lo[k + 1]; b += HTILE) {
                    tiles.push_back(make_uint4(a, qr, b, std::min<uint32_t>(HTILE, ce_lo[k + 1] - b)));
                    n_thin += pass == 0;
                }
            }
    lap("host: lists");
    DevBuf &dqcl = scratch[6], &dnl = scratch[7], &dql = scratch[8], &del = scratch[9], &dtl = scratch[10], &dqs = scratch[11], &dcl = scratch[13];
    if ((rc = dqcl.ensure(2 * (size_t)nq)) || (rc = dnl.ensure(2 * (size_t)npad)) || (rc = dql.ensure(4 * (size_t)nhq)) || (rc = del.ensure(4 * (size_t)nhe)) ||
        (rc = dtl.ensure(16 * tiles.size())) || (rc = dqs.ensure(sizeof(T) * (size_t)m * nhq)) || (rc = dcl.ensure(4 * (size_t)(K + 2)))) return rc;
    GS_HIP_CHECK(hipMemcpyAsync(dqcl.p, hqcl, 2 * (size_t)nq, hipMemcpyHostToDevice, c->stream));
    GS_HIP_CHECK(hipMemcpyAsync(dnl.p, hnl, 2 * (size_t)npad, hipMemcpyHostToDevice, c->stream));
    GS_HIP_CHECK(hipMemcpyAsync(dql.p, qlist.data(), 4 * (size_t)nhq, hipMemcpyHostToDevice, c->stream));
    GS_HIP_CHECK(hipMemcpyAsync(del.p, elist.data(), 4 * (size_t)nhe, hipMemcpyHostToDevice, c->stream));
    GS_HIP_CHECK(hipMemcpyAsync(dtl.p, tiles.data(), 16 * tiles.size(), hipMemcpyHostToDevice, c->stream));
    GS_HIP_CHECK(hipMemcpyAsync(dcl.p, cl_lo.data(), 4 * (size_t)(K + 2), hipMemcpyHostToDevice, c->stream));
    GS_HIP_CHECK(hipStreamSynchronize(c->stream));
    hipLaunchKernelGGL((k_query_cols_list<T>), dim3((nhq + 31) / 32, (m + 31) / 32), dim3(256), 0, c->stream, qrows, qstride, dql.as<uint32_t>(), nhq, m, dqs.as<T>());
    GS_HIP_CHECK(hipGetLastError());
    lap("uploads + sorted key copy");
    const bool inplace = getenv("GS_JOIN_INPLACE") ? atoi(getenv("GS_JOIN_INPLACE")) != 0 : nhe * 10 >= n;
    if ((rc = join_launch<KIND, T, true>(c, g, k0.as<T>(), nq, cols, colcap, n, JS0, m, out16, ld, stats, 0, false, dqcl.as<uint16_t>(), dnl.as<uint16_t>(), dqs.as<T>(), nhq,
                                         dcl.as<uint32_t>(), dql.as<uint32_t>(), dedup_below | (inplace ? 0x80000000u : 0u)))) return rc;
    {
        ProfScope ps(c, FAM_HAMMING);
        lap("cluster-aware join");
        if ((rc = hamming_blocks(c, KIND, m, qrows, qstride, rows, rstride, dtl.p, (uint32_t)tiles.size(), dql.as<uint32_t>(), del.as<uint32_t>(), out16, ld, n_thin))) return rc;
        lap("block compare");
    }
    return GS_OK;
}

uint64_t match_join_max_queries() { const char *e = getenv("GS_JOIN_MAXQ"); return e ? (uint64_t)std::max(1, std::min(4094, atoi(e))) : JQ_MAX; }

int match_join_counts(gs_ctx *c, int kind, uint32_t m, const void *qrows, uint64_t qstride, uint64_t nq, const void *cols, uint64_t colcap, uint64_t n,
                      uint16_t *out16, uint64_t ld, DevBuf *scratch, int *declined, unsigned long long *stats, bool init, uint64_t col0, const void *rows, uint64_t rstride)
{
    GS_REQUIRE(nq >= 1 && nq <= 4094 && m <= 65535 && (ld % 2) == 0 && ((uintptr_t)out16 % 4) == 0, GS_ERR_INVALID, "match_join_counts: bad shape");
    GS_REQUIRE((uint64_t)m * nq < ((uint64_t)1 << 31), GS_ERR_INVALID, "match_join_counts: batch too large");
    if (kind == GS_KIND_U64) return join_impl<GS_KIND_U64, uint64_t>(c, m, (const uint8_t *)qrows, qstride, (uint32_t)nq, cols, colcap, n, out16, ld, scratch, declined, stats, init, col0, rows, rstride);
    if (kind == GS_KIND_F32) return join_impl<GS_KIND_F32, uint32_t>(c, m, (const uint8_t *)qrows, qstride, (uint32_t)nq, cols, colcap, n, out16, ld, scratch, declined, stats, init, col0, rows, rstride);
    return join_impl<GS_KIND_U32, uint32_t>(c, m, (const uint8_t *)qrows, qstride, (uint32_t)nq, cols, colcap, n, out16, ld, scratch, declined, stats, init, col0, rows, rstride);
}

int rows_to_cols(gs_ctx *c, int kind, uint32_t m, const void *rows, uint64_t stride, uint64_t nrows, void *cols, uint64_t colcap, uint64_t first)
{
    if (nrows == 0) return GS_OK;
    dim3 g((uint32_t)((nrows + 31) / 32), (m + 31) / 32);
    if (kind == GS_KIND_U64) hipLaunchKernelGGL((k_rows_to_cols<uint64_t>), g, dim3(256), 0, c->stream, (const uint8_t *)rows, stride, nrows, m, (uint64_t *)cols, colcap, first, 0);
    else hipLaunchKernelGGL((k_rows_to_cols<uint32_t>), g, dim3(256), 0, c->stream, (const uint8_t *)rows, stride, nrows, m, (uint32_t *)cols, colcap, first, (int)(kind == GS_KIND_F32));
    GS_HIP_CHECK(hipGetLastError());
    return GS_OK;
}

}
```

Measured before the change: 53210.

## Merge up to eight join query batches into batched kernel launches

When the query set spans several join batches, dense_counts now passes groups of up to eight batches to one match_join_counts call. The query-column, heavy-scan, label and first-stage join kernels take a batch index in a grid dimension, and per-batch counters and pairs live in per-batch slices of scratch. The aim is to cut launch counts, host round trips and syncs per batch and to fill the GPU better with small batches. It costs more scratch and pinned memory per batch and makes the control flow considerably more complex.

```diff
diff --git a/gsearch_amd/csrc/gs_index.hip b/gsearch_amd/csrc/gs_index.hip
--- a/gsearch_amd/csrc/gs_index.hip
+++ b/gsearch_amd/csrc/gs_index.hip
@@ -2203,6 +2203,22 @@
     if ((rc = ensure_cols(ix, n))) return rc;
     if ((rc = ensure_stats(ix))) return rc;
     const uint64_t parts = (nq + match_join_max_queries() - 1) / match_join_max_queries(), jq = (nq + parts - 1) / parts;
+    const char *me = getenv("GS_JOIN_MERGE");
+    if (parts >= 2 && !ix->feed && !(me && !atoi(me))) {
+        const uint64_t group = jq * JOIN_BATCHES;
+        for (uint64_t g0 = 0; g0 < nq; g0 += group) {
+            const uint64_t ng = std::min<uint64_t>(group, nq - g0);
+            int declined[JOIN_BATCHES] = {};
+            if ((rc = match_join_counts(c, ix->ikind, ix->prm.m, qrows + g0 * ix->stride, ix->stride, ng, ix->cols.p, ix->cols_cap, n, out16 + g0 * ld, ld, ix->join_scratch,
+                                        declined, ix->stats.as<unsigned long long>(), true, 0, ix->data.p, ix->stride, jq))) return rc;
+            for (uint64_t q0 = g0, b = 0; q0 < g0 + ng; q0 += jq, b++) {
+                const uint64_t nb = std::min<uint64_t>(jq, g0 + ng - q0);
+                if (declined[b] &&
+                    (rc = hamming_qxc_strided(c, ix->ikind, ix->prm.m, qrows + q0 * ix->stride, nb, ix->stride, ix->data.p, n, ix->stride, nullptr, nullptr, out16 + q0 * ld, ld))) return rc;
+            }
+        }
+        return GS_OK;
+    }
     for (uint64_t q0 = 0; q0 < nq; q0 += jq) {
         const uint64_t nb = std::min<uint64_t>(jq, nq - q0);
         int declined = 0;
diff --git a/gsearch_amd/csrc/gs_internal.hpp b/gsearch_amd/csrc/gs_internal.hpp
--- a/gsearch_amd/csrc/gs_internal.hpp
+++ b/gsearch_amd/csrc/gs_internal.hpp
@@ -112,10 +112,10 @@
 
 struct DevBuf;
 uint64_t match_join_max_queries();
-enum { JOIN_SCRATCH = 16 };
+enum { JOIN_SCRATCH = 16, JOIN_BATCHES = 8 };
 int match_join_counts(gs_ctx *c, int kind, uint32_t m, const void *qrows, uint64_t qstride, uint64_t nq, const void *cols, uint64_t colcap, uint64_t n,
                       uint16_t *out16, uint64_t ld, DevBuf *scratch, int *declined = nullptr, unsigned long long *stats = nullptr, bool init = true, uint64_t col0 = 0,
-                      const void *rows = nullptr, uint64_t rstride = 0);
+                      const void *rows = nullptr, uint64_t rstride = 0, uint64_t jq = 0);
 int hamming_blocks(gs_ctx *c, int kind, uint32_t m, const void *Q, uint64_t strideQ_bytes, const void *C, uint64_t strideC_bytes, const void *items_dev,
                    uint32_t n_items, const uint32_t *qlist_dev, const uint32_t *clist_dev, uint16_t *out_cnt16, uint64_t ld_out, uint32_t n_thin = 0,
                    uint32_t *parts_out = nullptr);
diff --git a/gsearch_amd/csrc/gs_join.hip b/gsearch_amd/csrc/gs_join.hip
--- a/gsearch_amd/csrc/gs_join.hip
+++ b/gsearch_amd/csrc/gs_join.hip
@@ -41,10 +41,16 @@
     }
 }
 
+struct JoinSpan { uint32_t nq, jq; };
+__device__ __forceinline__ uint32_t span_q0(const JoinSpan sp, uint32_t b) { return b * sp.jq; }
+__device__ __forceinline__ uint32_t span_nq(const JoinSpan sp, uint32_t b) { const uint32_t r = sp.nq - b * sp.jq; return r < sp.jq ? r : sp.jq; }
+
 template <int KIND, typename T>
-__global__ __launch_bounds__(256) void k_query_cols(const uint8_t *__restrict__ rows, uint64_t stride, uint32_t nq, uint32_t m, T *__restrict__ qkey)
+__global__ __launch_bounds__(256) void k_query_cols(const uint8_t *__restrict__ rows, uint64_t stride, JoinSpan sp, uint32_t m, T *__restrict__ qkey)
 {
     __shared__ T tile[32][33];
+    const uint32_t q0 = span_q0(sp, blockIdx.z), nq = span_nq(sp, blockIdx.z);
+    rows += (uint64_t)q0 * stride; qkey += (uint64_t)m * q0;
     const uint32_t tx = threadIdx.x & 31, ty = threadIdx.x >> 5;
     const uint64_t r0 = (uint64_t)blockIdx.x * 32, s0 = (uint64_t)blockIdx.y * 32;
     for (uint32_t j = ty; j < 32; j += 8) {
@@ -104,13 +110,16 @@
 constexpr uint32_t JCL_MAX = 2047;
 constexpr int JWALK = 4;
 
+struct JoinBatch { const void *qkey; uint32_t *mm32; uint32_t nq, pad; };
+
 template <int KIND, typename T, int SR, bool CL>
 __global__ __launch_bounds__(JT, (sizeof(T) == 8 && SR == 1) ? 4 : 8) void k_match_join(const T *__restrict__ qkey, uint32_t nq, uint32_t log2p, const T *__restrict__ cols, uint64_t colcap, uint64_t n,
                                                     uint32_t slot_lo, uint32_t slot_hi, uint32_t slots_per_wg, uint32_t *__restrict__ mm32, uint64_t ld,
                                                     unsigned long long *__restrict__ stats, int chunk_major, uint64_t col0, const uint16_t *__restrict__ qcl,
                                                     const uint16_t *__restrict__ nodelab, const T *__restrict__ qs, uint32_t nh, const uint32_t *__restrict__ cl_lo,
-                                                    const uint32_t *__restrict__ qlist, uint32_t dedup_flags)
-{
+                                                    const uint32_t *__restrict__ qlist, uint32_t dedup_flags, const JoinBatch *__restrict__ bt)
+{
+    if constexpr (!CL) { if (bt) { const JoinBatch b = bt[blockIdx.z]; qkey = (const T *)b.qkey; nq = b.nq; mm32 = b.mm32; } }
     const uint32_t dedup_below = dedup_flags & 0x7FFFFFFFu;
     static_assert(JU == 4 && JN % JU == 0, "GS_SEL4 / pending mask are written for JU = 4");
     static_assert(!CL || SR == 1, "clusters: request batches only");
@@ -535,9 +544,12 @@
 constexpr uint32_t JDEDUP_MINQ = 2;
 
 constexpr uint32_t HS_STAGE = 3072;
-__global__ __launch_bounds__(256) void k_heavy_scan(const uint16_t *__restrict__ mat, uint64_t ld, uint32_t nq, uint64_t n, uint32_t m, uint2 *__restrict__ pairs,
-                                                    unsigned long long *__restrict__ ctr , uint64_t cap)
-{
+constexpr uint32_t JCTR = 8;
+__global__ __launch_bounds__(256) void k_heavy_scan(const uint16_t *__restrict__ mat, uint64_t ld, uint64_t n, uint32_t m, uint2 *__restrict__ pairs,
+                                                    unsigned long long *__restrict__ ctr , uint64_t cap, JoinSpan sp)
+{
+    const uint32_t nq = span_nq(sp, blockIdx.y);
+    mat += (uint64_t)span_q0(sp, blockIdx.y) * ld; pairs += (uint64_t)blockIdx.y * cap; ctr += (uint64_t)blockIdx.y * JCTR;
     __shared__ uint2 stage[HS_STAGE];
     __shared__ uint32_t sn;
     __shared__ unsigned long long sbase;
@@ -580,14 +592,16 @@
     for (int o = 32; o > 0; o >>= 1) tot += __shfl_down(tot, o);
     if ((threadIdx.x & 63) == 0 && tot) atomicAdd(&ctr[1], (unsigned long long)tot);
 }
-__global__ void k_label_init(uint32_t *__restrict__ labq, uint32_t nq, uint32_t *__restrict__ labe, uint64_t n)
+__global__ void k_label_init(uint32_t *__restrict__ labq, JoinSpan sp, uint32_t *__restrict__ labe, uint64_t n)
 {
     const uint64_t i = (uint64_t)blockIdx.x * blockDim.x + threadIdx.x;
-    if (i < nq) labq[i] = (uint32_t)i;
-    if (i < n) labe[i] = 0xFFFFFFFFu;
-}
-__global__ void k_label_prop(const uint2 *__restrict__ pairs, const unsigned long long *__restrict__ ctr, uint64_t cap, uint32_t *__restrict__ labq, uint32_t *__restrict__ labe)
-{
+    if (i < span_nq(sp, blockIdx.y)) labq[span_q0(sp, blockIdx.y) + i] = (uint32_t)i;
+    if (i < n) labe[(uint64_t)blockIdx.y * n + i] = 0xFFFFFFFFu;
+}
+__global__ void k_label_prop(const uint2 *__restrict__ pairs, const unsigned long long *__restrict__ ctr, uint64_t cap, uint32_t *__restrict__ labq, uint32_t *__restrict__ labe,
+                             JoinSpan sp, uint64_t n)
+{
+    pairs += (uint64_t)blockIdx.y * cap; ctr += (uint64_t)blockIdx.y * JCTR; labq += span_q0(sp, blockIdx.y); labe += (uint64_t)blockIdx.y * n;
     const uint64_t np = ctr[0] < cap ? ctr[0] : cap;
     for (uint64_t i = (uint64_t)blockIdx.x * blockDim.x + threadIdx.x; i < np; i += (uint64_t)gridDim.x * blockDim.x) {
         const uint2 p = pairs[i];
@@ -596,8 +610,10 @@
         if (l < b) atomicMin(&labe[p.x], l);
     }
 }
-__global__ void k_label_count(const uint32_t *__restrict__ labe, uint64_t n, uint32_t nq, uint32_t *__restrict__ cnt)
-{
+__global__ void k_label_count(const uint32_t *__restrict__ labe, uint64_t n, JoinSpan sp, uint32_t *__restrict__ cnt)
+{
+    labe += (uint64_t)blockIdx.y * n; cnt += span_q0(sp, blockIdx.y);
+    const uint32_t nq = span_nq(sp, blockIdx.y);
     for (uint64_t e = (uint64_t)blockIdx.x * blockDim.x + threadIdx.x; e < n; e += (uint64_t)gridDim.x * blockDim.x) { const uint32_t l = labe[e]; if (l < nq) atomicAdd(&cnt[l], 1u); }
 }
 template <typename T>
@@ -621,7 +637,7 @@
 template <int KIND, typename T, bool CL>
 static int join_launch(gs_ctx *c, const JoinGeom &g, const T *qkey, uint32_t nq, const void *cols, uint64_t colcap, uint64_t n, uint32_t slot_lo, uint32_t slot_hi,
                        uint16_t *out16, uint64_t ld, unsigned long long *stats, uint64_t col0, bool few_blocks, const uint16_t *qcl, const uint16_t *nodelab, const T *qs,
-                       uint32_t nh, const uint32_t *cl_lo, const uint32_t *qlist, uint32_t dedup_below = 0)
+                       uint32_t nh, const uint32_t *cl_lo, const uint32_t *qlist, uint32_t dedup_below = 0, const JoinBatch *batches = nullptr, uint32_t nbatches = 1)
 {
     const uint32_t ms = slot_hi - slot_lo, chunks = g.chunks;
     uint32_t blocks = std::max<uint32_t>(1, std::min<uint32_t>((16 * c->n_cu) / chunks, std::max<uint32_t>(ms / 32, (2 * c->n_cu) / chunks)));
@@ -631,7 +647,7 @@
     const uint32_t slots_per_wg = (ms + blocks - 1) / blocks;
     const int chunk_major = getenv("GS_JOIN_CHUNK_MAJOR") ? atoi(getenv("GS_JOIN_CHUNK_MAJOR")) : ((nq >= 1024 && chunks >= 16) ? 1 : 0);
     const uint32_t nblk = (ms + slots_per_wg - 1) / slots_per_wg;
-    dim3 jg(chunk_major ? nblk : chunks, chunk_major ? chunks : nblk);
+    dim3 jg(chunk_major ? nblk : chunks, chunk_major ? chunks : nblk, nbatches);
     int sr = 1;
     if (!CL) {
         if (4 * g.lds1 <= 80 * 1024 && slots_per_wg >= 8) sr = 4; else if (2 * g.lds1 <= 80 * 1024 && slots_per_wg >= 4) sr = 2;
@@ -644,7 +660,7 @@
         auto kern = KERN;                                                                                                                             \
         if (lds > 48 * 1024) GS_HIP_CHECK(hipFuncSetAttribute((const void *)kern, hipFuncAttributeMaxDynamicSharedMemorySize, (int)lds));             \
         hipLaunchKernelGGL(kern, jg, dim3(JT), lds, c->stream, qkey, nq, g.log2p, (const T *)cols, colcap, n, slot_lo, slot_hi, slots_per_wg, (uint32_t *)out16, ld, \
-                           stats, chunk_major, col0, qcl, nodelab, qs, nh, cl_lo, qlist, dedup_below);                                                             \
+                           stats, chunk_major, col0, qcl, nodelab, qs, nh, cl_lo, qlist, dedup_below, batches);                                                    \
     } while (0)
     if (CL) GS_JOIN_GO((k_match_join<KIND, T, 1, CL>));
     else if (sr == 4) GS_JOIN_GO((k_match_join<KIND, T, 4, false>));
@@ -684,37 +700,53 @@
     return GS_OK;
 }
 
+struct JoinPlan {
+    uint64_t npairs = 0, pair_cap = 0, nhe = 0;
+    uint32_t K = 0, ntiles = 0, nhq = 0, dedup_below = 1;
+    bool sample = false;
+    std::vector<uint32_t> cq, ce_, cid;
+};
+
 template <int KIND, typename T>
-static int join_impl(gs_ctx *c, uint32_t m, const uint8_t *qrows, uint64_t qstride, uint32_t nq, const void *cols, uint64_t colcap, uint64_t n, uint16_t *out16,
+static int join_impl(gs_ctx *c, uint32_t m, const uint8_t *qrows, uint64_t qstride, uint32_t nq_all, uint32_t jq, const void *cols, uint64_t colcap, uint64_t n, uint16_t *out16,
                      uint64_t ld, DevBuf *scratch , int *declined, unsigned long long *stats, bool init, uint64_t col0,
                      const void *rows, uint64_t rstride)
 {
     int rc;
-    if (declined) *declined = 0;
-    const size_t items = (size_t)m * nq;
+    const uint32_t B = (nq_all + jq - 1) / jq;
+    const JoinSpan span{nq_all, jq};
+    auto q0_of = [&](uint32_t b) { return b * jq; };
+    auto nq_of = [&](uint32_t b) { return std::min<uint32_t>(jq, nq_all - b * jq); };
+    if (declined) for (uint32_t b = 0; b < B; b++) declined[b] = 0;
     DevBuf &k0 = scratch[0];
-    if ((rc = k0.ensure(sizeof(T) * items))) return rc;
-    if (init) GS_HIP_CHECK(hipMemsetD16Async((hipDeviceptr_t)out16, (unsigned short)m, (size_t)nq * ld, c->stream));
-    dim3 tg((nq + 31) / 32, (m + 31) / 32);
-    hipLaunchKernelGGL((k_query_cols<KIND, T>), tg, dim3(256), 0, c->stream, qrows, qstride, nq, m, k0.as<T>());
+    if ((rc = k0.ensure(sizeof(T) * (size_t)m * nq_all))) return rc;
+    auto qkey_of = [&](uint32_t b) { return k0.as<T>() + (size_t)m * q0_of(b); };
+    auto out_of = [&](uint32_t b) { return out16 + (uint64_t)q0_of(b) * ld; };
+    if (init) GS_HIP_CHECK(hipMemsetD16Async((hipDeviceptr_t)out16, (unsigned short)m, (size_t)nq_all * ld, c->stream));
+    dim3 tg((jq + 31) / 32, (m + 31) / 32, B);
+    hipLaunchKernelGGL((k_query_cols<KIND, T>), tg, dim3(256), 0, c->stream, qrows, qstride, span, m, k0.as<T>());
     GS_HIP_CHECK(hipGetLastError());
+    const uint32_t nq_max = jq, nq_min = nq_of(B - 1);
     JoinGeom g;
     g.log2p = 6;
-    while (g.log2p < (uint32_t)JP_MAX_LOG2 && (double)(1u << g.log2p) * 0.4 < (double)nq) g.log2p++;
+    while (g.log2p < (uint32_t)JP_MAX_LOG2 && (double)(1u << g.log2p) * 0.4 < (double)nq_max) g.log2p++;
     g.chunks = (uint32_t)((n + (uint64_t)JT * JN - 1) / ((uint64_t)JT * JN));
     g.lds1 = (sizeof(T) + 4) * ((size_t)1 << g.log2p) + ((size_t)1 << JB_LOG2) / 8;
     g.ldsq = (size_t)(JT / 64) * 64 * (sizeof(T) == 4 ? 8 : 16);
     const bool may_decline = declined && m >= 64 && n >= 4096;
     const char *ce = getenv("GS_JOIN_CLUSTER");
-    bool cluster = declined && init && col0 == 0 && rows && nq >= 256 && n >= 8192 && m >= 16 * JS0 && (ld % 8) == 0 && !(ce && !atoi(ce)) && !getenv("GS_JOIN_DECLINE");
+    bool cluster = declined && init && col0 == 0 && rows && nq_min >= 256 && n >= 8192 && m >= 16 * JS0 && (ld % 8) == 0 && !(ce && !atoi(ce)) && !getenv("GS_JOIN_DECLINE");
     if (ce && atoi(ce) == 2) cluster = declined && init && col0 == 0 && rows && m >= 2 * JS0 && (ld % 8) == 0;
     if (!cluster) {
-        if (may_decline) {
-            int dec = 0;
-            if ((rc = join_sample_declines<KIND, T>(c, g, m, k0.as<T>(), nq, cols, colcap, n, scratch, &dec))) return rc;
-            if (dec) { *declined = 1; return GS_OK; }
-        }
-        return join_launch<KIND, T, false>(c, g, k0.as<T>(), nq, cols, colcap, n, 0, m, out16, ld, stats, col0, false, nullptr, nullptr, nullptr, 0, nullptr, nullptr);
+        for (uint32_t b = 0; b < B; b++) {
+            if (may_decline) {
+                int dec = 0;
+                if ((rc = join_sample_declines<KIND, T>(c, g, m, qkey_of(b), nq_of(b), cols, colcap, n, scratch, &dec))) return rc;
+                if (dec) { declined[b] = 1; continue; }
+            }
+            if ((rc = join_launch<KIND, T, false>(c, g, qkey_of(b), nq_of(b), cols, colcap, n, 0, m, out_of(b), ld, stats, col0, false, nullptr, nullptr, nullptr, 0, nullptr, nullptr))) return rc;
+        }
+        return GS_OK;
     }
     const bool verbose = getenv("GS_JOIN_VERBOSE") != nullptr;
     const bool times = getenv("GS_JOIN_TIMES") != nullptr;
@@ -728,138 +760,192 @@
     };
     lap("query columns + memset");
     DevBuf &pairs = scratch[2], &ctr = scratch[3], &labq = scratch[4], &labe = scratch[5];
-    uint64_t pair_cap = JPAIR_CAP;
-    DevBuf &lcnt = scratch[14];
-    if ((rc = pairs.ensure(pair_cap * 8)) || (rc = ctr.ensure(64)) || (rc = labq.ensure(4 * (size_t)nq)) || (rc = labe.ensure(4 * (size_t)n)) || (rc = lcnt.ensure(4 * (size_t)nq))) return rc;
-    pair_cap = std::max<uint64_t>(pair_cap, pairs.bytes / 8);
-    if ((rc = join_launch<KIND, T, false>(c, g, k0.as<T>(), nq, cols, colcap, n, 0, JS0, out16, ld, stats, 0, true, nullptr, nullptr, nullptr, 0, nullptr, nullptr))) return rc;
+    DevBuf &lcnt = scratch[14], &dbt = scratch[15];
+    if ((rc = pairs.ensure(JPAIR_CAP * 8 * B)) || (rc = ctr.ensure(8 * JCTR * B)) || (rc = labq.ensure(4 * (size_t)nq_all)) || (rc = labe.ensure(4 * (size_t)n * B)) ||
+        (rc = lcnt.ensure(4 * (size_t)nq_all)) || (rc = dbt.ensure(2 * JOIN_BATCHES * sizeof(JoinBatch)))) return rc;
+    uint64_t cap_each = pairs.bytes / 8 / B;
+    if (const char *pc = getenv("GS_JOIN_PAIR_CAP")) cap_each = std::min<uint64_t>(cap_each, (uint64_t)std::max(1, atoi(pc)));
+    const size_t pin_head = 64 * (size_t)JOIN_BATCHES + 2 * JOIN_BATCHES * sizeof(JoinBatch) + 8 * (size_t)nq_all;
+    const size_t pin_each = (4 * (size_t)n + 2 * ((size_t)nq_max + 8 + (size_t)g.chunks * JT * JN) + 63) & ~(size_t)63;
+    uint8_t *pin = (uint8_t *)pinned_pool(c)->ensure(PIN_JOIN, pin_head + 64 + pin_each * B);
+    GS_REQUIRE(pin, GS_ERR_HIP, "match-join: pinned staging buffer");
+    JoinBatch *hbt = (JoinBatch *)(pin + 64 * (size_t)JOIN_BATCHES);
+    uint32_t *hlq_all = (uint32_t *)(hbt + 2 * JOIN_BATCHES), *hcn_all = hlq_all + nq_all;
+    auto hc_of = [&](uint32_t b) { return (unsigned long long *)(pin + 64 * (size_t)b); };
+    auto hle_of = [&](uint32_t b) { return (uint32_t *)(pin + ((pin_head + 63) & ~(size_t)63) + pin_each * b); };
+    auto join_many = [&](const std::vector<uint32_t> &bs, uint32_t at, uint32_t slot_lo, uint32_t slot_hi, bool few_blocks) -> int {
+        if (bs.size() == 1)
+            return join_launch<KIND, T, false>(c, g, qkey_of(bs[0]), nq_of(bs[0]), cols, colcap, n, slot_lo, slot_hi, out_of(bs[0]), ld, stats, 0, few_blocks, nullptr, nullptr, nullptr, 0, nullptr, nullptr);
+        for (size_t i = 0; i < bs.size(); i++) hbt[at + i] = JoinBatch{qkey_of(bs[i]), (uint32_t *)out_of(bs[i]), nq_of(bs[i]), 0u};
+        GS_HIP_CHECK(hipMemcpyAsync(dbt.as<JoinBatch>() + at, hbt + at, bs.size() * sizeof(JoinBatch), hipMemcpyHostToDevice, c->stream));
+        return join_launch<KIND, T, false>(c, g, (const T *)nullptr, nq_max, cols, colcap, n, slot_lo, slot_hi, nullptr, ld, stats, 0, few_blocks, nullptr, nullptr, nullptr, 0, nullptr, nullptr,
+                                           0, dbt.as<JoinBatch>() + at, (uint32_t)bs.size());
+    };
+    std::vector<uint32_t> all_b(B);
+    for (uint32_t b = 0; b < B; b++) all_b[b] = b;
+    if ((rc = join_many(all_b, 0, 0, JS0, true))) return rc;
     lap("phase 0 (first slots)");
-    uint8_t *pin = (uint8_t *)pinned_pool(c)->ensure(PIN_JOIN, 64 + 4 * (2 * (size_t)nq + n) + 2 * ((size_t)nq + 8 + (size_t)g.chunks * JT * JN) + 64);
-    GS_REQUIRE(pin, GS_ERR_HIP, "match-join: pinned staging buffer");
-    unsigned long long *hc = (unsigned long long *)pin;
-    uint32_t *hlq = (uint32_t *)(pin + 64), *hcn = hlq + nq, *hle = hcn + nq;
-    for (int attempt = 0;; attempt++) {
-        GS_HIP_CHECK(hipMemsetAsync(ctr.p, 0, 64, c->stream));
-        hipLaunchKernelGGL(k_heavy_scan, dim3(c->n_cu * 8), dim3(256), 0, c->stream, out16, ld, nq, n, m, pairs.as<uint2>(), ctr.as<unsigned long long>(), pair_cap);
+    auto scan_and_label = [&](uint32_t b0, uint32_t cnt, uint64_t cap) -> int {
+        const uint32_t q0 = q0_of(b0), nqs = std::min<uint32_t>(nq_all - q0, cnt * jq);
+        const JoinSpan sp{nqs, jq};
+        unsigned long long *dctr = ctr.as<unsigned long long>() + (size_t)JCTR * b0;
+        uint32_t *dlq = labq.as<uint32_t>() + q0, *dle = labe.as<uint32_t>() + (size_t)n * b0, *dcn = lcnt.as<uint32_t>() + q0;
+        GS_HIP_CHECK(hipMemsetAsync(dctr, 0, 8 * (size_t)JCTR * cnt, c->stream));
+        hipLaunchKernelGGL(k_heavy_scan, dim3(c->n_cu * 8, cnt), dim3(256), 0, c->stream, out_of(b0), ld, n, m, pairs.as<uint2>(), dctr, cap, sp);
         lap("heavy scan");
-        hipLaunchKernelGGL(k_label_init, dim3((uint32_t)((std::max<uint64_t>(n, nq) + 255) / 256)), dim3(256), 0, c->stream, labq.as<uint32_t>(), nq, labe.as<uint32_t>(), n);
+        hipLaunchKernelGGL(k_label_init, dim3((uint32_t)((std::max<uint64_t>(n, jq) + 255) / 256), cnt), dim3(256), 0, c->stream, dlq, sp, dle, n);
         for (int it = 0; it < 6; it++)
-            hipLaunchKernelGGL(k_label_prop, dim3(c->n_cu * 4), dim3(256), 0, c->stream, pairs.as<uint2>(), ctr.as<unsigned long long>(), pair_cap, labq.as<uint32_t>(), labe.as<uint32_t>());
-        GS_HIP_CHECK(hipMemsetAsync(lcnt.p, 0, 4 * (size_t)nq, c->stream));
-        hipLaunchKernelGGL(k_label_count, dim3(c->n_cu * 2), dim3(256), 0, c->stream, labe.as<uint32_t>(), n, nq, lcnt.as<uint32_t>());
+            hipLaunchKernelGGL(k_label_prop, dim3(c->n_cu * 4, cnt), dim3(256), 0, c->stream, pairs.as<uint2>(), dctr, cap, dlq, dle, sp, n);
+        GS_HIP_CHECK(hipMemsetAsync(dcn, 0, 4 * (size_t)nqs, c->stream));
+        hipLaunchKernelGGL(k_label_count, dim3(c->n_cu * 2, cnt), dim3(256), 0, c->stream, dle, n, sp, dcn);
         GS_HIP_CHECK(hipGetLastError());
-        GS_HIP_CHECK(hipMemcpyAsync(hc, ctr.p, 16, hipMemcpyDeviceToHost, c->stream));
-        GS_HIP_CHECK(hipMemcpyAsync(hlq, labq.p, 4 * (size_t)nq, hipMemcpyDeviceToHost, c->stream));
-        GS_HIP_CHECK(hipMemcpyAsync(hcn, lcnt.p, 4 * (size_t)nq, hipMemcpyDeviceToHost, c->stream));
+        GS_HIP_CHECK(hipMemcpyAsync(hc_of(b0), dctr, 8 * (size_t)JCTR * cnt, hipMemcpyDeviceToHost, c->stream));
+        GS_HIP_CHECK(hipMemcpyAsync(hlq_all + q0, dlq, 4 * (size_t)nqs, hipMemcpyDeviceToHost, c->stream));
+        GS_HIP_CHECK(hipMemcpyAsync(hcn_all + q0, dcn, 4 * (size_t)nqs, hipMemcpyDeviceToHost, c->stream));
+        return GS_OK;
+    };
+    if ((rc = scan_and_label(0, B, cap_each))) return rc;
+    GS_HIP_CHECK(hipStreamSynchronize(c->stream));
+    lap("labels + query labels down");
+    std::vector<JoinPlan> plans(B);
+    for (uint32_t b = 0; b < B; b++) {
+        plans[b].pair_cap = cap_each;
+        const uint64_t want = hc_of(b)[0];
+        if (want <= cap_each || want > JPAIR_MAX) continue;
+        if (want * 8 + 4096 > pairs.bytes && pairs.alloc((size_t)want * 8 + 4096) != GS_OK) { (void)hipGetLastError(); (void)pairs.alloc(JPAIR_CAP * 8 * B); continue; }
+        plans[b].pair_cap = want + 512;
+        if ((rc = scan_and_label(b, 1, plans[b].pair_cap))) return rc;
         GS_HIP_CHECK(hipStreamSynchronize(c->stream));
-        lap("labels + query labels down");
-        if (hc[0] <= pair_cap || attempt || hc[0] > JPAIR_MAX) break;
-        if (pairs.alloc((size_t)hc[0] * 8 + 4096) != GS_OK) { (void)hipGetLastError(); (void)pairs.alloc(JPAIR_CAP * 8); pair_cap = JPAIR_CAP; break; }
-        pair_cap = hc[0] + 512;
-    }
-    const uint64_t npairs = hc[0];
-    std::vector<uint32_t> cq(nq, 0), ce_(nq, 0), cid(nq, 0);
-    uint32_t K = 0, ntiles = 0, nhq = 0, dedup_below = 1;
-    uint64_t nhe = 0;
-    const uint32_t minq = getenv("GS_JOIN_CLUSTER_MINQ") ? (uint32_t)std::max(2, atoi(getenv("GS_JOIN_CLUSTER_MINQ"))) : (ce && atoi(ce) == 2 ? 2u : 12u);
-    const uint64_t minpairs = getenv("GS_JOIN_CLUSTER_MINPAIRS") ? (uint64_t)atoll(getenv("GS_JOIN_CLUSTER_MINPAIRS")) : 128;
-    auto is_cluster = [&](uint32_t l) { return cq[l] >= minq || (cq[l] >= 2 && (uint64_t)(cq[l] - 1) * hcn[l] >= minpairs); };
-    const uint64_t min_scaled0 = (uint64_t)((double)nq * 32.0 * (double)n / 3.0e5);
-    const uint64_t min_saved0 = getenv("GS_JOIN_CLUSTER_MIN") ? (uint64_t)atoll(getenv("GS_JOIN_CLUSTER_MIN")) : (ce && atoi(ce) == 2 ? 0 : std::max<uint64_t>((uint64_t)nq * 8, min_scaled0));
-    bool any = false;
-    if (npairs <= pair_cap) {
-        for (uint32_t q = 0; q < nq; q++) if (hlq[q] < nq) ++cq[hlq[q]];
-        uint64_t est = 0;
-        for (uint32_t l = 0; l < nq; l++) if (cq[l] && hcn[l] && is_cluster(l)) { any = true; est += (uint64_t)(cq[l] - 1) * hcn[l]; }
-        if (est < min_saved0) any = false;
-    }
-    if (any) {
-        GS_HIP_CHECK(hipMemcpyAsync(hle, labe.p, 4 * (size_t)n, hipMemcpyDeviceToHost, c->stream));
+        lap("labels + query labels down (list regrown)");
+    }
+    const double tile_rate = KIND == GS_KIND_U64 ? 1.4e13 : 1.6e13;
+    std::vector<uint32_t> plain;
+    for (uint32_t b = 0; b < B; b++) {
+        JoinPlan &pl = plans[b];
+        const uint32_t nq = nq_of(b);
+        const unsigned long long *hc = hc_of(b);
+        const uint32_t *hlq = hlq_all + q0_of(b), *hcn = hcn_all + q0_of(b);
+        uint32_t *hle = hle_of(b);
+        const uint64_t npairs = pl.npairs = hc[0], pair_cap = pl.pair_cap;
+        std::vector<uint32_t> &cq = pl.cq, &ce_ = pl.ce_, &cid = pl.cid;
+        cq.assign(nq, 0); ce_.assign(nq, 0); cid.assign(nq, 0);
+        uint32_t &K = pl.K, &ntiles = pl.ntiles, &nhq = pl.nhq, &dedup_below = pl.dedup_below;
+        uint64_t &nhe = pl.nhe;
+        const uint32_t minq = getenv("GS_JOIN_CLUSTER_MINQ") ? (uint32_t)std::max(2, atoi(getenv("GS_JOIN_CLUSTER_MINQ"))) : (ce && atoi(ce) == 2 ? 2u : 12u);
+        const uint64_t minpairs = getenv("GS_JOIN_CLUSTER_MINPAIRS") ? (uint64_t)atoll(getenv("GS_JOIN_CLUSTER_MINPAIRS")) : 128;
+        auto is_cluster = [&](uint32_t l) { return cq[l] >= minq || (cq[l] >= 2 && (uint64_t)(cq[l] - 1) * hcn[l] >= minpairs); };
+        const uint64_t min_scaled0 = (uint64_t)((double)nq * 32.0 * (double)n / 3.0e5);
+        const uint64_t min_saved0 = getenv("GS_JOIN_CLUSTER_MIN") ? (uint64_t)atoll(getenv("GS_JOIN_CLUSTER_MIN")) : (ce && atoi(ce) == 2 ? 0 : std::max<uint64_t>((uint64_t)nq * 8, min_scaled0));
+        bool any = false;
+        if (npairs <= pair_cap) {
+            for (uint32_t q = 0; q < nq; q++) if (hlq[q] < nq) ++cq[hlq[q]];
+            uint64_t est = 0;
+            for (uint32_t l = 0; l < nq; l++) if (cq[l] && hcn[l] && is_cluster(l)) { any = true; est += (uint64_t)(cq[l] - 1) * hcn[l]; }
+            if (est < min_saved0) any = false;
+        }
+        if (any) {
+            GS_HIP_CHECK(hipMemcpyAsync(hle, labe.as<uint32_t>() + (size_t)n * b, 4 * (size_t)n, hipMemcpyDeviceToHost, c->stream));
+            GS_HIP_CHECK(hipStreamSynchronize(c->stream));
+            for (uint64_t e = 0; e < n; e++) if (hle[e] < nq) ce_[hle[e]]++;
+            std::vector<uint32_t> order;
+            for (uint32_t l = 0; l < nq; l++) if (ce_[l] >= 1 && is_cluster(l)) order.push_back(l);
+            auto tiles_of = [&](uint32_t l) { return ((cq[l] + HTILE - 1) / HTILE) * ((ce_[l] + HTILE - 1) / HTILE); };
+            std::sort(order.begin(), order.end(), [&](uint32_t a, uint32_t b) { const uint32_t ta = tiles_of(a), tb = tiles_of(b); return ta != tb ? ta < tb : a < b; });
+            std::vector<uint32_t> chosen;
+            for (uint32_t l : order) {
+                if (chosen.size() >= JCL_MAX || ntiles + tiles_of(l) > JTILE_CAP) break;
+                chosen.push_back(l); ntiles += tiles_of(l); nhq += cq[l]; nhe += ce_[l];
+            }
+            const uint32_t dq = getenv("GS_JOIN_DEDUP_MINQ") ? (uint32_t)std::max(2, atoi(getenv("GS_JOIN_DEDUP_MINQ"))) : JDEDUP_MINQ;
+            std::stable_sort(chosen.begin(), chosen.end(), [&](uint32_t a, uint32_t b) { return (cq[a] >= dq) > (cq[b] >= dq); });
+            for (uint32_t l : chosen) { cid[l] = ++K; if (cq[l] >= dq) dedup_below = K + 1; }
+        }
+        uint64_t saved_pairs = 0;
+        for (uint32_t l = 0; l < nq; l++) if (cid[l]) saved_pairs += (uint64_t)(cq[l] - 1) * ce_[l];
+        const uint64_t min_scaled = (uint64_t)((double)nq * 32.0 * (double)n / 3.0e5);
+        const uint64_t min_saved = getenv("GS_JOIN_CLUSTER_MIN") ? (uint64_t)atoll(getenv("GS_JOIN_CLUSTER_MIN")) : (ce && atoi(ce) == 2 ? 0 : std::max<uint64_t>((uint64_t)nq * 8, min_scaled));
+        if (verbose)
+            fprintf(stderr, "[GS_JOIN] nq=%u n=%llu heavy pairs %llu (matches in the first %u slots %llu): %u clusters, %u queries x %llu nodes in %u tiles, %llu pairs off the atomics%s\n", nq,
+                    (unsigned long long)n, (unsigned long long)npairs, JS0, hc[1], K, nhq, (unsigned long long)nhe, ntiles, (unsigned long long)saved_pairs,
+                    K && saved_pairs < min_saved ? " - not worth the cluster-aware pass" : "");
+        if (K && saved_pairs < min_saved) K = 0;
+        if (K == 0) {
+            const double t_tile = (double)((nq + 127) / 128 * 128) * (double)n * (double)m / tile_rate;
+            pl.sample = may_decline && (npairs > pair_cap || (double)hc[1] * ((double)m / JS0) / 1.6e10 > 0.5 * t_tile);
+            if (!pl.sample) plain.push_back(b);
+        }
+    }
+    lap("host: components");
+    if (!plain.empty() && (rc = join_many(plain, JOIN_BATCHES, JS0, m, false))) return rc;
+    lap("plain join (merged)");
+    for (uint32_t b = 0; b < B; b++) {
+        JoinPlan &pl = plans[b];
+        const uint32_t nq = nq_of(b), K = pl.K, nhq = pl.nhq, dedup_below = pl.dedup_below;
+        const uint64_t nhe = pl.nhe;
+        const uint8_t *qrows_b = qrows + (uint64_t)q0_of(b) * qstride;
+        if (K == 0) {
+            if (!pl.sample) continue;
+            int dec = 0;
+            if ((rc = join_sample_declines<KIND, T>(c, g, m, qkey_of(b), nq, cols, colcap, n, scratch, &dec))) return rc;
+            if (dec) { declined[b] = 1; continue; }
+            if ((rc = join_launch<KIND, T, false>(c, g, qkey_of(b), nq, cols, colcap, n, JS0, m, out_of(b), ld, stats, 0, false, nullptr, nullptr, nullptr, 0, nullptr, nullptr))) return rc;
+            continue;
+        }
+        const std::vector<uint32_t> &cq = pl.cq, &ce_ = pl.ce_, &cid = pl.cid;
+        const uint32_t *hlq = hlq_all + q0_of(b);
+        uint32_t *hle = hle_of(b);
+        std::vector<uint32_t> cl_lo(K + 2, 0), ce_lo(K + 2, 0);
+        for (uint32_t l = 0; l < nq; l++) if (cid[l]) { cl_lo[cid[l] + 1] = cq[l]; ce_lo[cid[l] + 1] = ce_[l]; }
+        for (uint32_t k = 1; k <= K + 1; k++) { cl_lo[k] += cl_lo[k - 1]; ce_lo[k] += ce_lo[k - 1]; }
+        std::vector<uint32_t> qlist(nhq), elist(nhe), fq(cl_lo.begin(), cl_lo.end()), fe(ce_lo.begin(), ce_lo.end());
+        const uint64_t npad = (uint64_t)g.chunks * JT * JN;
+        uint16_t *hqcl = (uint16_t *)(hle + n), *hnl = hqcl + ((nq + 3) & ~3u);
+        for (uint32_t q = 0; q < nq; q++) { const uint32_t l = hlq[q]; hqcl[q] = 0; if (l < nq && cid[l]) { hqcl[q] = (uint16_t)cid[l]; qlist[fq[cid[l]]++] = q; } }
+        memset(hnl, 0, 2 * npad);
+        for (uint64_t e = 0; e < n; e++) {
+            const uint32_t l = hle[e];
+            if (l < nq && cid[l]) {
+                const uint64_t ch = e / (JT * JN), w = e % (JT * JN), i = w / JT, ln = w % JT;
+                hnl[((ch * (JN / JU) + i / JU) * JT + ln) * JU + i % JU] = (uint16_t)cid[l];
+                elist[fe[cid[l]]++] = (uint32_t)e;
+            }
+        }
+        std::vector<uint4> tiles;
+        tiles.reserve(pl.ntiles);
+        uint32_t n_thin = 0;
+        for (int pass = 0; pass < 2; pass++)
+            for (uint32_t k = 1; k <= K; k++)
+                for (uint32_t a = cl_lo[k]; a < cl_lo[k + 1]; a += HTILE) {
+                    const uint32_t qr = std::min<uint32_t>(HTILE, cl_lo[k + 1] - a);
+                    if ((qr <= (uint32_t)HTQ) != (pass == 0)) continue;
+                    for (uint32_t e = ce_lo[k]; e < ce_lo[k + 1]; e += HTILE) {
+                        tiles.push_back(make_uint4(a, qr, e, std::min<uint32_t>(HTILE, ce_lo[k + 1] - e)));
+                        n_thin += pass == 0;
+                    }
+                }
+        lap("host: lists");
+        DevBuf &dqcl = scratch[6], &dnl = scratch[7], &dql = scratch[8], &del = scratch[9], &dtl = scratch[10], &dqs = scratch[11], &dcl = scratch[13];
+        if ((rc = dqcl.ensure(2 * (size_t)nq)) || (rc = dnl.ensure(2 * (size_t)npad)) || (rc = dql.ensure(4 * (size_t)nhq)) || (rc = del.ensure(4 * (size_t)nhe)) ||
+            (rc = dtl.ensure(16 * tiles.size())) || (rc = dqs.ensure(sizeof(T) * (size_t)m * nhq)) || (rc = dcl.ensure(4 * (size_t)(K + 2)))) return rc;
+        GS_HIP_CHECK(hipMemcpyAsync(dqcl.p, hqcl, 2 * (size_t)nq, hipMemcpyHostToDevice, c->stream));
+        GS_HIP_CHECK(hipMemcpyAsync(dnl.p, hnl, 2 * (size_t)npad, hipMemcpyHostToDevice, c->stream));
+        GS_HIP_CHECK(hipMemcpyAsync(dql.p, qlist.data(), 4 * (size_t)nhq, hipMemcpyHostToDevice, c->stream));
+        GS_HIP_CHECK(hipMemcpyAsync(del.p, elist.data(), 4 * (size_t)nhe, hipMemcpyHostToDevice, c->stream));
+        GS_HIP_CHECK(hipMemcpyAsync(dtl.p, tiles.data(), 16 * tiles.size(), hipMemcpyHostToDevice, c->stream));
+        GS_HIP_CHECK(hipMemcpyAsync(dcl.p, cl_lo.data(), 4 * (size_t)(K + 2), hipMemcpyHostToDevice, c->stream));
         GS_HIP_CHECK(hipStreamSynchronize(c->stream));
-        for (uint64_t e = 0; e < n; e++) if (hle[e] < nq) ce_[hle[e]]++;
-        std::vector<uint32_t> order;
-        for (uint32_t l = 0; l < nq; l++) if (ce_[l] >= 1 && is_cluster(l)) order.push_back(l);
-        auto tiles_of = [&](uint32_t l) { return ((cq[l] + HTILE - 1) / HTILE) * ((ce_[l] + HTILE - 1) / HTILE); };
-        std::sort(order.begin(), order.end(), [&](uint32_t a, uint32_t b) { const uint32_t ta = tiles_of(a), tb = tiles_of(b); return ta != tb ? ta < tb : a < b; });
-        std::vector<uint32_t> chosen;
-        for (uint32_t l : order) {
-            if (chosen.size() >= JCL_MAX || ntiles + tiles_of(l) > JTILE_CAP) break;
-            chosen.push_back(l); ntiles += tiles_of(l); nhq += cq[l]; nhe += ce_[l];
-        }
-        const uint32_t dq = getenv("GS_JOIN_DEDUP_MINQ") ? (uint32_t)std::max(2, atoi(getenv("GS_JOIN_DEDUP_MINQ"))) : JDEDUP_MINQ;
-        std::stable_sort(chosen.begin(), chosen.end(), [&](uint32_t a, uint32_t b) { return (cq[a] >= dq) > (cq[b] >= dq); });
-        for (uint32_t l : chosen) { cid[l] = ++K; if (cq[l] >= dq) dedup_below = K + 1; }
-    }
-    uint64_t saved_pairs = 0;
-    for (uint32_t l = 0; l < nq; l++) if (cid[l]) saved_pairs += (uint64_t)(cq[l] - 1) * ce_[l];
-    const uint64_t min_scaled = (uint64_t)((double)nq * 32.0 * (double)n / 3.0e5);
-    const uint64_t min_saved = getenv("GS_JOIN_CLUSTER_MIN") ? (uint64_t)atoll(getenv("GS_JOIN_CLUSTER_MIN")) : (ce && atoi(ce) == 2 ? 0 : std::max<uint64_t>((uint64_t)nq * 8, min_scaled));
-    if (verbose)
-        fprintf(stderr, "[GS_JOIN] nq=%u n=%llu heavy pairs %llu (matches in the first %u slots %llu): %u clusters, %u queries x %llu nodes in %u tiles, %llu pairs off the atomics%s\n", nq,
-                (unsigned long long)n, (unsigned long long)npairs, JS0, hc[1], K, nhq, (unsigned long long)nhe, ntiles, (unsigned long long)saved_pairs,
-                K && saved_pairs < min_saved ? " - not worth the cluster-aware pass" : "");
-    if (K && saved_pairs < min_saved) K = 0;
-    lap("host: components");
-    if (K == 0) {
-        const double t_tile = (double)((nq + 127) / 128 * 128) * (double)n * (double)m / (KIND == GS_KIND_U64 ? 1.4e13 : 1.6e13);
-        if (may_decline && (npairs > pair_cap || (double)hc[1] * ((double)m / JS0) / 1.6e10 > 0.5 * t_tile)) {
-            int dec = 0;
-            if ((rc = join_sample_declines<KIND, T>(c, g, m, k0.as<T>(), nq, cols, colcap, n, scratch, &dec))) return rc;
-            if (dec) { *declined = 1; return GS_OK; }
-        }
-        return join_launch<KIND, T, false>(c, g, k0.as<T>(), nq, cols, colcap, n, JS0, m, out16, ld, stats, 0, false, nullptr, nullptr, nullptr, 0, nullptr, nullptr);
-    }
-    std::vector<uint32_t> cl_lo(K + 2, 0), ce_lo(K + 2, 0);
-    for (uint32_t l = 0; l < nq; l++) if (cid[l]) { cl_lo[cid[l] + 1] = cq[l]; ce_lo[cid[l] + 1] = ce_[l]; }
-    for (uint32_t k = 1; k <= K + 1; k++) { cl_lo[k] += cl_lo[k - 1]; ce_lo[k] += ce_lo[k - 1]; }
-    std::vector<uint32_t> qlist(nhq), elist(nhe), fq(cl_lo.begin(), cl_lo.end()), fe(ce_lo.begin(), ce_lo.end());
-    const uint64_t npad = (uint64_t)g.chunks * JT * JN;
-    uint16_t *hqcl = (uint16_t *)(hle + n), *hnl = hqcl + ((nq + 3) & ~3u);
-    for (uint32_t q = 0; q < nq; q++) { const uint32_t l = hlq[q]; hqcl[q] = 0; if (l < nq && cid[l]) { hqcl[q] = (uint16_t)cid[l]; qlist[fq[cid[l]]++] = q; } }
-    memset(hnl, 0, 2 * npad);
-    for (uint64_t e = 0; e < n; e++) {
-        const uint32_t l = hle[e];
-        if (l < nq && cid[l]) {
-            const uint64_t ch = e / (JT * JN), w = e % (JT * JN), i = w / JT, ln = w % JT;
-            hnl[((ch * (JN / JU) + i / JU) * JT + ln) * JU + i % JU] = (uint16_t)cid[l];
-            elist[fe[cid[l]]++] = (uint32_t)e;
-        }
-    }
-    std::vector<uint4> tiles;
-    tiles.reserve(ntiles);
-    uint32_t n_thin = 0;
-    for (int pass = 0; pass < 2; pass++)
-        for (uint32_t k = 1; k <= K; k++)
-            for (uint32_t a = cl_lo[k]; a < cl_lo[k + 1]; a += HTILE) {
-                const uint32_t qr = std::min<uint32_t>(HTILE, cl_lo[k + 1] - a);
-                if ((qr <= (uint32_t)HTQ) != (pass == 0)) continue;
-                for (uint32_t b = ce_lo[k]; b < ce_lo[k + 1]; b += HTILE) {
-                    tiles.push_back(make_uint4(a, qr, b, std::min<uint32_t>(HTILE, ce_lo[k + 1] - b)));
-                    n_thin += pass == 0;
-                }
-            }
-    lap("host: lists");
-    DevBuf &dqcl = scratch[6], &dnl = scratch[7], &dql = scratch[8], &del = scratch[9], &dtl = scratch[10], &dqs = scratch[11], &dcl = scratch[13];
-    if ((rc = dqcl.ensure(2 * (size_t)nq)) || (rc = dnl.ensure(2 * (size_t)npad)) || (rc = dql.ensure(4 * (size_t)nhq)) || (rc = del.ensure(4 * (size_t)nhe)) ||
-        (rc = dtl.ensure(16 * tiles.size())) || (rc = dqs.ensure(sizeof(T) * (size_t)m * nhq)) || (rc = dcl.ensure(4 * (size_t)(K + 2)))) return rc;
-    GS_HIP_CHECK(hipMemcpyAsync(dqcl.p, hqcl, 2 * (size_t)nq, hipMemcpyHostToDevice, c->stream));
-    GS_HIP_CHECK(hipMemcpyAsync(dnl.p, hnl, 2 * (size_t)npad, hipMemcpyHostToDevice, c->stream));
-    GS_HIP_CHECK(hipMemcpyAsync(dql.p, qlist.data(), 4 * (size_t)nhq, hipMemcpyHostToDevice, c->stream));
-    GS_HIP_CHECK(hipMemcpyAsync(del.p, elist.data(), 4 * (size_t)nhe, hipMemcpyHostToDevice, c->stream));
-    GS_HIP_CHECK(hipMemcpyAsync(dtl.p, tiles.data(), 16 * tiles.size(), hipMemcpyHostToDevice, c->stream));
-    GS_HIP_CHECK(hipMemcpyAsync(dcl.p, cl_lo.data(), 4 * (size_t)(K + 2), hipMemcpyHostToDevice, c->stream));
-    GS_HIP_CHECK(hipStreamSynchronize(c->stream));
-    hipLaunchKernelGGL((k_query_cols_list<T>), dim3((nhq + 31) / 32, (m + 31) / 32), dim3(256), 0, c->stream, qrows, qstride, dql.as<uint32_t>(), nhq, m, dqs.as<T>());
-    GS_HIP_CHECK(hipGetLastError());
-    lap("uploads + sorted key copy");
-    const bool inplace = getenv("GS_JOIN_INPLACE") ? atoi(getenv("GS_JOIN_INPLACE")) != 0 : nhe * 10 >= n;
-    if ((rc = join_launch<KIND, T, true>(c, g, k0.as<T>(), nq, cols, colcap, n, JS0, m, out16, ld, stats, 0, false, dqcl.as<uint16_t>(), dnl.as<uint16_t>(), dqs.as<T>(), nhq,
-                                         dcl.as<uint32_t>(), dql.as<uint32_t>(), dedup_below | (inplace ? 0x80000000u : 0u)))) return rc;
-    {
-        ProfScope ps(c, FAM_HAMMING);
-        lap("cluster-aware join");
-        if ((rc = hamming_blocks(c, KIND, m, qrows, qstride, rows, rstride, dtl.p, (uint32_t)tiles.size(), dql.as<uint32_t>(), del.as<uint32_t>(), out16, ld, n_thin))) return rc;
-        lap("block compare");
+        hipLaunchKernelGGL((k_query_cols_list<T>), dim3((nhq + 31) / 32, (m + 31) / 32), dim3(256), 0, c->stream, qrows_b, qstride, dql.as<uint32_t>(), nhq, m, dqs.as<T>());
+        GS_HIP_CHECK(hipGetLastError());
+        lap("uploads + sorted key copy");
+        const bool inplace = getenv("GS_JOIN_INPLACE") ? atoi(getenv("GS_JOIN_INPLACE")) != 0 : nhe * 10 >= n;
+        if ((rc = join_launch<KIND, T, true>(c, g, qkey_of(b), nq, cols, colcap, n, JS0, m, out_of(b), ld, stats, 0, false, dqcl.as<uint16_t>(), dnl.as<uint16_t>(), dqs.as<T>(), nhq,
+                                             dcl.as<uint32_t>(), dql.as<uint32_t>(), dedup_below | (inplace ? 0x80000000u : 0u)))) return rc;
+        {
+            ProfScope ps(c, FAM_HAMMING);
+            lap("cluster-aware join");
+            if ((rc = hamming_blocks(c, KIND, m, qrows_b, qstride, rows, rstride, dtl.p, (uint32_t)tiles.size(), dql.as<uint32_t>(), del.as<uint32_t>(), out_of(b), ld, n_thin))) return rc;
+            lap("block compare");
+        }
     }
     return GS_OK;
 }
@@ -867,13 +953,16 @@
 uint64_t match_join_max_queries() { const char *e = getenv("GS_JOIN_MAXQ"); return e ? (uint64_t)std::max(1, std::min(4094, atoi(e))) : JQ_MAX; }
 
 int match_join_counts(gs_ctx *c, int kind, uint32_t m, const void *qrows, uint64_t qstride, uint64_t nq, const void *cols, uint64_t colcap, uint64_t n,
-                      uint16_t *out16, uint64_t ld, DevBuf *scratch, int *declined, unsigned long long *stats, bool init, uint64_t col0, const void *rows, uint64_t rstride)
-{
-    GS_REQUIRE(nq >= 1 && nq <= 4094 && m <= 65535 && (ld % 2) == 0 && ((uintptr_t)out16 % 4) == 0, GS_ERR_INVALID, "match_join_counts: bad shape");
-    GS_REQUIRE((uint64_t)m * nq < ((uint64_t)1 << 31), GS_ERR_INVALID, "match_join_counts: batch too large");
-    if (kind == GS_KIND_U64) return join_impl<GS_KIND_U64, uint64_t>(c, m, (const uint8_t *)qrows, qstride, (uint32_t)nq, cols, colcap, n, out16, ld, scratch, declined, stats, init, col0, rows, rstride);
-    if (kind == GS_KIND_F32) return join_impl<GS_KIND_F32, uint32_t>(c, m, (const uint8_t *)qrows, qstride, (uint32_t)nq, cols, colcap, n, out16, ld, scratch, declined, stats, init, col0, rows, rstride);
-    return join_impl<GS_KIND_U32, uint32_t>(c, m, (const uint8_t *)qrows, qstride, (uint32_t)nq, cols, colcap, n, out16, ld, scratch, declined, stats, init, col0, rows, rstride);
+                      uint16_t *out16, uint64_t ld, DevBuf *scratch, int *declined, unsigned long long *stats, bool init, uint64_t col0, const void *rows, uint64_t rstride,
+                      uint64_t jq)
+{
+    if (jq == 0 || jq > nq) jq = nq;
+    GS_REQUIRE(nq >= 1 && jq >= 1 && jq <= 4094 && (nq + jq - 1) / jq <= JOIN_BATCHES && m <= 65535 && (ld % 2) == 0 && ((uintptr_t)out16 % 4) == 0, GS_ERR_INVALID,
+               "match_join_counts: bad shape");
+    GS_REQUIRE((uint64_t)m * jq < ((uint64_t)1 << 31), GS_ERR_INVALID, "match_join_counts: batch too large");
+    if (kind == GS_KIND_U64) return join_impl<GS_KIND_U64, uint64_t>(c, m, (const uint8_t *)qrows, qstride, (uint32_t)nq, (uint32_t)jq, cols, colcap, n, out16, ld, scratch, declined, stats, init, col0, rows, rstride);
+    if (kind == GS_KIND_F32) return join_impl<GS_KIND_F32, uint32_t>(c, m, (const uint8_t *)qrows, qstride, (uint32_t)nq, (uint32_t)jq, cols, colcap, n, out16, ld, scratch, declined, stats, init, col0, rows, rstride);
+    return join_impl<GS_KIND_U32, uint32_t>(c, m, (const uint8_t *)qrows, qstride, (uint32_t)nq, (uint32_t)jq, cols, colcap, n, out16, ld, scratch, declined, stats, init, col0, rows, rstride);
 }
 
 int rows_to_cols(gs_ctx *c, int kind, uint32_t m, const void *rows, uint64_t stride, uint64_t nrows, void *cols, uint64_t colcap, uint64_t first)
```

Result: faster. 54090, median of 6 (+1.6%).
